# hitbc/deSAMBA

Measured on AMD Instinct MI355X. Metric: classified reads/s (50 kbp ONT reads, viral index), higher is better.
Workload: dtype u8/u64 integer

## Files before the change

__graft_entry__.py:

```python
import os
import subprocess
import sys

ROOT = os.path.dirname(os.path.abspath(__file__))
CSRC = os.path.join(ROOT, "desamba_amd", "csrc")
LIB = os.path.join(ROOT, "desamba_amd", "libdesamba_amd.so")
HIPCC = os.environ.get("HIPCC", "/opt/rocm/bin/hipcc")


def _run(cmd, cwd=None):
    print("+", " ".join(cmd), flush=True)
    subprocess.check_call(cmd, cwd=cwd)


def _newer(target, sources):
    if not os.path.exists(target):
        return False
    t = os.path.getmtime(target)
    return all(os.path.getmtime(s) <= t for s in sources)


def build():
    inc = os.path.join(ROOT, "include", "desamba_amd.h")
    H = lambda *names: [os.path.join(CSRC, f) for f in names] + [inc]
# ... 12 lines not shown
            o = os.path.join(objdir, src + (".o" if ku is None else ".k%d.o" % ku))
            if not _newer(o, [os.path.join(CSRC, src)] + hdrs) or os.environ.get("DSB_HIPCC_FLAGS"):
                jobs.append([HIPCC] + flags + ([] if ku is None else ["-DDSB_KUNIT=%d" % ku]) + ["-c", os.path.join(CSRC, src), "-o", o])
            objs.append(o)
    stage_dir = os.path.join(ROOT, "tests", "stage")
    stage_so = os.path.join(stage_dir, "libdsbstage.so")
    stage_src = os.path.join(stage_dir, "dsb_stage.hip")
    stage_forms = os.path.join(stage_dir, "dsb_stage_forms.h")
    if os.path.exists(stage_src) and os.path.exists(stage_forms) and (
            not _newer(stage_so, [stage_src, stage_forms] + H("dsb_classify_dev.h", "dsb_wave.h", "dsb_device.h")) or os.environ.get("DSB_HIPCC_FLAGS")):
        jobs.append([HIPCC] + flags + ["-I" + CSRC, "-I" + stage_dir, "-shared", "-o", stage_so, stage_src])
    if jobs:
        from concurrent.futures import ThreadPoolExecutor
        with ThreadPoolExecutor(max_workers=max(1, min(len(jobs), os.cpu_count() or 1))) as ex:
            list(ex.map(_run, jobs))
    stale = os.path.join(objdir, "dsb_gpu.hip.o")
    if os.path.exists(stale):
        os.remove(stale)
    deps = [os.path.join(CSRC, f) for f in ("dsb_classify_dev.h", "dsb_wave.h", "dsb_device.h", "dsb_host.h", "dsb_probe.h", "dsb_fastq_scan.h", "dsb_seed_scan.h", "dsb_build_impl.h", "dsb_build_host.h", "dsb_sam_fields.h")] + [inc]
    if not _newer(LIB, objs):
        _run([HIPCC, "--offload-arch=gfx950", "-shared", "-fPIC", "-o", LIB] + objs + ["-lz"])
    cli = os.path.join(ROOT, "desamba_amd", "bin", "deSAMBA")
    cli_src = os.path.join(CSRC, "desamba_main.c")
    ana_src = os.path.join(CSRC, "desamba_analysis.c")
    if os.path.exists(cli_src) and not _newer(cli, [cli_src, ana_src, LIB, os.path.join(CSRC, "dsb_fastq_scan.h")]):
        os.makedirs(os.path.dirname(cli), exist_ok=True)
        _run(["gcc", "-O2", "-std=gnu99", "-I" + os.path.join(ROOT, "include"), "-o", cli, cli_src, ana_src,
              "-L" + os.path.join(ROOT, "desamba_amd"), "-ldesamba_amd", "-Wl,-rpath,$ORIGIN/..", "-lpthread", "-lz", "-ldl"])
    sim = os.path.join(ROOT, "tools", "readsim")
    if not _newer(sim, [sim + ".c"]):
        _run(["gcc", "-O2", "-o", sim, sim + ".c", "-lm"])
    gen = os.path.join(ROOT, "tools", "libreadgen.so")
    if not _newer(gen, [os.path.join(ROOT, "tools", "readgen.c")]):
        _run(["gcc", "-O2", "-shared", "-fPIC", "-o", gen, os.path.join(ROOT, "tools", "readgen.c"), "-lpthread", "-lm"])
    gb = os.path.join(ROOT, "tools", "gather_bench")
    if not _newer(gb, [gb + ".hip"]):
        _run([HIPCC, "-O3", "--offload-arch=gfx950", gb + ".hip", "-o", gb])
    _run(["make", "-s", "-C", os.path.join(ROOT, "oracle"), "tools", "port", "ref", "ref_ubfree"])
    emu = os.path.join(ROOT, "tests", "emu", "libdsbemu.so")
    emu_src = os.path.join(ROOT, "tests", "emu", "emu_classify.cpp")
    emu_b = os.path.join(ROOT, "tests", "emu", "libdsbemu_build.so")
    emu_b_src = os.path.join(ROOT, "tests", "emu", "emu_build.cpp")
    if not _newer(emu_b, [emu_b_src] + H("dsb_build_impl.h", "dsb_build_parts.h", "dsb_build_host.h", "dsb_probe.h")):
        _run(["g++", "-std=c++17", "-O2", "-fno-strict-aliasing", "-fPIC", "-shared", "-I" + CSRC, "-I" + os.path.join(ROOT, "include"), "-o", emu_b, emu_b_src, "-lz"])
    emu_dir = os.path.join(ROOT, "tests", "emu")
    if os.path.exists(stage_forms):
        deps = deps + [stage_forms]
    if not _newer(emu, [emu_src, os.path.join(emu_dir, "dsb_emu_shim.h")] + deps):
        _run(["g++", "-std=c++17", "-O2", "-fno-strict-aliasing", "-fPIC", "-shared", "-DDSB_HOST_EMU", "-I" + CSRC, "-I" + os.path.join(ROOT, "include"), "-I" + emu_dir,
              "-o", emu, emu_src, os.path.join(CSRC, "dsb_index.cpp")])
    emu64 = os.path.join(emu_dir, "libdsbemu64.so")
    if not _newer(emu64, [emu_src, os.path.join(emu_dir, "dsb_emu_shim.h"), os.path.join(emu_dir, "emu_simt.cpp")] + deps):
        _run([os.path.join(emu_dir, "build_emu64.sh")])
    sys.path.insert(0, ROOT)
    import desamba_amd
    L = desamba_amd.lib()
    for name in desamba_amd.EXPORTS:
        getattr(L, name)
    print("build ok:", L.dsb_version().decode(), flush=True)


def demo_dir():
    d = os.path.join(ROOT, "data")
    if not os.access(d if os.path.isdir(d) else ROOT, os.W_OK):
        import tempfile
        d = os.path.join(tempfile.gettempdir(), "desamba_amd_data_%d" % os.getuid())
    d = os.path.join(d, "demo")
    subprocess.check_call([os.path.join(ROOT, "tools", "make_demo_index.sh"), d], stdout=sys.stderr)
    return d


def smoke():
    sys.path.insert(0, ROOT)
    sys.path.insert(0, os.path.join(ROOT, "tests"))
    import desamba_amd as D
    import oracle_lib as O
    d = demo_dir()
    idx = D.Index(os.path.join(d, "index"))
    ctx = D.Ctx(idx, 0)
    recs = D.read_fastq(os.path.join(d, "ERR1050068.fastq"), 32)
    reads = D.make_reads(recs)
    res = ctx.classify(reads)
    ora = O.Oracle(os.path.join(d, "index"))
    hist = 0
    for i, (name, seq, qual) in enumerate(recs):
        exp = ora.classify(seq, hist)
        hist = max(hist, len(seq))
        rr = res.reads[i]
        got = [res.hits[rr.first + k].key() for k in range(rr.n)]
        assert got == exp, "smoke: read %d differs from the oracle: %r vs %r" % (i, got, exp)
    t = ctx.timing()
    print("smoke ok: 32 reads bit-exact vs oracle; kernels ms: encode %.3f probe %.3f classify %.3f" % (t.encode_ms, t.seed_probe_ms, t.classify_ms), flush=True)
    ctx.close(); idx.close()


if __name__ == "__main__":
    build()
    if len(sys.argv) > 1 and sys.argv[1] == "smoke":
        smoke()
```

desamba_amd/__init__.py:

```python
import ctypes as C
import os

_HERE = os.path.dirname(os.path.abspath(__file__))
LIB_PATH = os.environ.get("DSB_LIB_PATH", os.path.join(_HERE, "libdesamba_amd.so"))

DSB_OK, DSB_EIO, DSB_ENODEV, DSB_ENOMEM, DSB_EINVAL, DSB_ECAP = 0, -1, -2, -3, -4, -5


class DsbOpts(C.Structure):
    _fields_ = [("L_min_matching", C.c_int), ("min_score", C.c_int), ("max_sec_N", C.c_int), ("n_slots", C.c_int),
                ("max_read_len", C.c_uint32), ("max_batch_reads", C.c_uint32), ("input_slots", C.c_int), ("reserved", C.c_int), ("max_batch_bases", C.c_uint64)]


class DsbRead(C.Structure):
    _fields_ = [("name", C.c_char_p), ("seq", C.c_char_p), ("qual", C.c_char_p), ("len", C.c_uint32)]


class DsbHit(C.Structure):
    _fields_ = [("ref_ID", C.c_uint32), ("t_st", C.c_uint32), ("t_ed", C.c_uint32), ("q_st", C.c_uint32), ("q_ed", C.c_uint32),
                ("sum_score", C.c_uint32), ("indel", C.c_uint32), ("direction", C.c_uint8), ("primary", C.c_uint8),
                ("pri_index", C.c_uint8), ("pad", C.c_uint8)]

    def key(self):
        return (self.ref_ID, self.t_st, self.t_ed, self.q_st, self.q_ed, self.sum_score, self.direction, self.primary, self.pri_index)


class DsbReadResult(C.Structure):
    _fields_ = [("first", C.c_uint32), ("n", C.c_uint32), ("status", C.c_int32), ("fast", C.c_uint32), ("device_us", C.c_uint32), ("n_anc", C.c_uint32)]


class DsbResult(C.Structure):
    _fields_ = [("reads", C.POINTER(DsbReadResult)), ("hits", C.POINTER(DsbHit)), ("n_hits", C.c_size_t)]


class DsbSeed(C.Structure):
    _fields_ = [("offset", C.c_uint32), ("len", C.c_uint32), ("top", C.c_uint8), ("pad", C.c_uint8 * 3)]


class DsbTiming(C.Structure):
    _fields_ = [("encode_ms", C.c_float), ("seed_probe_ms", C.c_float), ("classify_ms", C.c_float), ("total_ms", C.c_float),
                ("windows", C.c_uint64), ("probes_t1", C.c_uint64), ("bases", C.c_uint64),
                ("order_ms", C.c_float), ("tail_ms", C.c_float), ("n_early", C.c_uint32), ("n_retry", C.c_uint32),
                ("n_regrow", C.c_uint32), ("seed_scan", C.c_uint32),
                ("n_occ", C.c_uint64), ("n_mem", C.c_uint64), ("n_sa", C.c_uint64), ("ref_bases", C.c_uint64),
                ("main_occ", C.c_uint64), ("main_mem", C.c_uint64), ("main_sa", C.c_uint64), ("main_ref_bases", C.c_uint64),
                ("n_heavy_mw", C.c_uint32), ("n_requeue", C.c_uint32), ("upload_bytes", C.c_uint64),
                ("anc_pool_asked", C.c_uint64), ("anc_pool_cap", C.c_uint64)]


class DsbBuildStats(C.Structure):
    _fields_ = [(n, C.c_uint64) for n in ("n_bases", "n_refs", "n_kmer", "n_unitig", "n_rows")] + \
               [(n, C.c_double) for n in ("parse_s", "sort_s", "graph_s", "walk_s", "rows_s", "tables_s", "write_s", "total_s")] + \
               [(n, C.c_uint64) for n in ("budget_bytes", "peak_device_bytes")] + \
               [(n, C.c_uint32) for n in ("ranges_kmers", "ranges_unitig_numbers", "ranges_rows", "ranges_exist")] + \
               [("spilled_bytes", C.c_uint64)]


class DsbReadTaxon(C.Structure):
    _fields_ = [("taxid", C.c_uint32), ("score", C.c_uint32), ("len", C.c_uint32), ("mapq", C.c_uint8), ("flags", C.c_uint8), ("pad", C.c_uint16)]


DSB_TAXON_CLASSIFIED, DSB_TAXON_HOST = 1, 2


class DsbRefCoverage(C.Structure):
    _fields_ = [("numreads", C.c_uint64), ("covbases", C.c_uint64), ("aligned_bases", C.c_uint64), ("mapq_sum", C.c_uint64)]


COVERAGE_FIELDS = ("numreads", "covbases", "aligned_bases", "mapq_sum")


class DsbEmOpts(C.Structure):
    _fields_ = [("max_iter", C.c_uint32), ("reserved", C.c_uint32), ("tol", C.c_double)]


class DsbAbundanceSummary(C.Structure):
    _fields_ = [("reads", C.c_uint64), ("classified", C.c_uint64), ("classes", C.c_uint64), ("iterations", C.c_uint32),
                ("converged", C.c_uint32), ("max_change", C.c_double), ("min_permille", C.c_uint32), ("reserved", C.c_uint32)]


ABUNDANCE_DTYPE = [("numreads", "<u8"), ("uniqreads", "<u8"), ("est_reads", "<f8"), ("read_share", "<f8"), ("copy_share", "<f8")]


class DsbReadLca(C.Structure):
    _fields_ = [("taxid", C.c_uint32), ("score", C.c_uint32), ("n_pass", C.c_uint32), ("depth", C.c_uint16), ("flags", C.c_uint8), ("pad", C.c_uint8)]


DSB_LCA_CLASSIFIED, DSB_LCA_NO_TAXON, DSB_LCA_AMBIGUOUS = 1, 2, 4
LCA_DTYPE = [("taxid", "<u4"), ("score", "<u4"), ("n_pass", "<u4"), ("depth", "<u2"), ("flags", "u1"), ("pad", "u1")]
TAXON_COUNT_DTYPE = [("taxid", "<u4"), ("pad", "<u4"), ("clade_reads", "<u8"), ("direct_reads", "<u8")]


class DsbLcaSummary(C.Structure):
    _fields_ = [("reads", C.c_uint64), ("classified", C.c_uint64), ("no_taxon", C.c_uint64), ("ambiguous", C.c_uint64),
                ("min_permille", C.c_uint32), ("reserved", C.c_uint32)]


LCA_SUMMARY_FIELDS = ("reads", "classified", "no_taxon", "ambiguous", "min_permille")


# ... 722 lines not shown
```

desamba_amd/csrc/dsb_classify_dev.h:

```cpp
#include "dsb_device.h"

#ifndef DSB_GROUP
#define DSB_GROUP 64
#endif
#ifndef DSB_NS
#define DSB_NS dsb_g64
#endif

#ifndef DSB_DEV_COMMON
#define DSB_DEV_COMMON
#define MAXV(a,b) (((a) > (b))?(a):(b))
#define MINV(a,b) (((a) < (b))?(a):(b))
#define ABSV(a) (((a) > 0)?(a): (- (a)))
#define ABS_U(a,b) (((a) > (b))?((a) - (b)): ((b) - (a)))
#define D_FORWARD 1u
#define D_REVERSE 0u
#define D_U64MAX 0xffffffffffffffffULL
#define SPENT(w) (++(w).steps > (w).step_limit)
#define LSPENT(l) (++(l).lsteps > (l).step_limit)
#define TICK(w, k) do { if ((w).dbg) { uint64_t _t = DSB_CLOCK(); (w).tacc[k] += _t - (w).tlast; (w).tlast = _t; } } while (0)
#ifdef DSB_TIMERS
#define SUB0(w) do { if ((w).dbg) (w).tsub = DSB_CLOCK(); } while (0)
#define SUB1(w, k) do { if ((w).dbg) (w).tacc[k] += DSB_CLOCK() - (w).tsub; } while (0)
#define TX0(w, v) uint64_t v = (w).dbg ? DSB_CLOCK() : 0
#define TX1(w, k, v) do { if ((w).dbg) (w).tx[k] += DSB_CLOCK() - (v); } while (0)
#define TXC(w, k) do { if ((w).dbg) (w).tx[k] += 1; } while (0)
#else
#define SUB0(w) do { } while (0)
#define SUB1(w, k) do { } while (0)
#define TX0(w, v) do { } while (0)
#define TX1(w, k, v) do { } while (0)
#define TXC(w, k) do { } while (0)
#endif
#define MARK(w, code) do { if ((w).dbg && DSB_LANE == 0) { (w).dbg[0] = (code); (w).dbg[1] = (w).steps; } } while (0)
#ifdef DSB_LDS_DIET
#define DSB_WTAB_SLOTS 2176u
#else
#define DSB_WTAB_SLOTS 3072u
#endif
#define DSB_WTAB_MAXQ 2048u
#define DSB_WTAB_EMPTY 0xffffffffu
#endif

#ifndef DSB_BOOST_IF_HEAVY
#define DSB_BOOST_PREDS 300000u
#define DSB_MIDDLE_HEAVY_MIN 16384u
#ifndef DSB_LANE_STEPS
#define DSB_LANE_STEPS 256u
#endif
#define DSB_BOOST_IF_HEAVY(w) do { if (!(w).boosted && (w).dp_preds > DSB_BOOST_PREDS) { dsb_setprio3(); (w).boosted = 1; } } while (0)
#endif
#define DSB_HEAVY_CHECK(w) do { if ((w).heavy_limit && (w).dp_preds > (w).heavy_limit) { (w).status |= DSB_ST_HEAVY; (w).steps = (w).step_limit; } } while (0)

namespace DSB_NS {

#ifdef DSB_HOST_EMU
#include "dsb_emu_shim.h"
#else
#include "dsb_wave.h"
#endif

struct Cnt { lds_u32 *c; uint32_t uni; };
DV void cnt_add(const Cnt &k, int which, uint32_t v)
{
	if (k.uni && DSB_LANE != 0) return;
	lds_add(k.c + which, v);
}

#define DSB_MW_MAXW 8
#ifndef DSB_MW_MIN_PREDS
#define DSB_MW_MIN_PREDS 2048
#endif
struct DsbMw {
	uint32_t cmd;
	uint32_t n0, K;
	const DsbSms *sms;
	uint32_t nd_t[8], nd_q[8], nd_l[8];
	uint32_t cut[2][DSB_MW_MAXW];
	int32_t best[DSB_MW_MAXW][8];
};

#define DSB_DPB 8
struct DpBatch { uint32_t n0, K; int old_best[DSB_DPB]; uint32_t nd_t[DSB_DPB], nd_q[DSB_DPB], nd_l[DSB_DPB]; };
typedef DSB_LDS_AS DpBatch DpBatchL;

struct SDir { DsbSeed *seed_v; uint32_t l_seed_v; uint8_t *bin_read; const uint64_t *bits; uint32_t direction, total_score; };
struct SDirV { DsbSeed *seed_v; uint8_t *bin_read; uint32_t direction; };

struct WCtx {
	DsbXP x;
	uint8_t *bin; uint32_t L;
	DsbSeed *seeds;
	DsbMw *mw; int n_waves;
	const uint64_t *pk[2];
	DsbSeed *pre_seeds; const DsbSeedInfo *pre_info;
	DsbAnchor *anc, *anc_tmp; uint32_t n_anc, anc_cap;
	uint32_t anc_cap_main, hit_cap, step_limit;
	DsbAnchor *lane_anc; uint64_t *lane_spset; uint32_t *top_idx;
	DsbChain *hit, *hit_tmp; uint32_t n_hit;
	DsbSms *sms; uint32_t n_sms;
	uint32_t *wtab;
	DsbScHash *sc;
	DsbMem *mem_slow;
	uint64_t *spset;
	int *score_v;
	uint64_t *sortkey; uint32_t *sortidx;
	uint8_t *win_mid, *win_right, *win_left;
	uint32_t *red;
	uint32_t *round_info;
	uint32_t dp_preds;
	uint32_t heavy_limit;
	DpBatchL *dpb;
	uint4 *ring;
	int status; int max_read_l;
	int stage; int boosted; uint32_t sp_gen;
	Cnt k;
	uint32_t steps, lsteps; volatile uint32_t *dbg; uint64_t tacc[14], tlast, tsub, tx[10];
	SDir sd[2];
};
typedef DSB_LDS_AS WCtx WCtxL;
typedef DSB_LDS_AS SDir SDirL;
DV void sdir_set(SDirL *d, DsbSeed *seed_v, uint32_t l_seed_v, uint8_t *bin_read, const uint64_t *bits, uint32_t direction, uint32_t total_score)
{
	d->seed_v = seed_v; d->l_seed_v = l_seed_v; d->bin_read = bin_read; d->bits = bits; d->direction = direction; d->total_score = total_score;
}
DV void sdir_swap(SDirL *a, SDirL *b)
{
	DsbSeed *sv = a->seed_v; const uint32_t n = a->l_seed_v; uint8_t *br = a->bin_read; const uint64_t *bi = a->bits; const uint32_t di = a->direction, ts = a->total_score;
	sdir_set(a, b->seed_v, b->l_seed_v, b->bin_read, b->bits, b->direction, b->total_score);
	sdir_set(b, sv, n, br, bi, di, ts);
}
#define WK(w) (Cnt{(w).k.c, (w).k.uni})
struct LCtx { DsbAnchor *anc; uint32_t n_anc, anc_cap; uint64_t *spset; int status; uint32_t lsteps, step_limit, sp_gen; Cnt k; };
DV LCtx lctx_main(WCtxL &w)
{
	LCtx l; l.anc = w.anc; l.n_anc = w.n_anc; l.anc_cap = w.anc_cap; l.spset = w.spset; l.status = w.status; l.lsteps = w.lsteps; l.step_limit = w.step_limit;
	l.sp_gen = w.sp_gen; l.k.c = w.k.c; l.k.uni = w.k.uni;
	return l;
}
DV void lctx_done(WCtxL &w, const LCtx &l) { w.n_anc = l.n_anc; w.status = l.status; w.lsteps = l.lsteps; w.sp_gen = l.sp_gen; }

DV bool dsb_serial_lane() { wave_sync(); return DSB_LANE == 0; }
#define DSB_SERIAL(w) if (dsb_serial_lane())
DV void serial_end(WCtxL &) { wave_sync(); }

DV uint64_t d_hash64_1(uint64_t key)
{
	key = (~key + (key << 21)); key = key ^ key >> 24; key = ((key + (key << 3)) + (key << 8));
	key = key ^ key >> 14; key = ((key + (key << 2)) + (key << 4)); key = key ^ key >> 28; key = (key + (key << 31));
	return key;
}
DV uint64_t d_hash64_2(uint64_t key)
{
// ... 1728 lines not shown
DV void sdp_limits(const DsbSms &cs, uint32_t &lim_q, uint32_t &lim_t)
{
	if (MODE == 2) { lim_q = cs.q_pos + cs.len - 6 + 9 - 1; lim_t = cs.t_pos + cs.len - 6 + 9 - 1; }
	else { lim_q = cs.q_pos + 6; lim_t = cs.t_pos + 6; }
}
template <int MODE>
DV void sdp_judge(const DsbSms &cs, const DsbSms &ps, uint32_t lim_q, uint32_t lim_t, bool &skip, bool &brk, int &ns)
{
	brk = false; ns = 0;
	if (MODE == 2) {
		skip = (ps.q_pos < lim_q) || (ps.t_pos < lim_t);
		if (!skip) brk = (lim_t + 600 < ps.t_pos);
		if (!skip && !brk) {
			int indel = ps.q_pos - ps.t_pos - (lim_q - lim_t); int ai = ABSV(indel);
			if (ai > 200) skip = true;
			else {
				ns = ps.score + cs.len - (ai >> 3);
				if (lim_q + 6 > ps.q_pos || lim_t + 6 > ps.t_pos) { int oq = lim_q + 6 - ps.q_pos, ot = lim_t + 6 - ps.t_pos; ns -= MAXV(oq, ot); }
			}
		}
	} else {
		int pre_q_ed = ps.q_pos + ps.len + 9 - 1, pre_t_ed = ps.t_pos + ps.len + 9 - 1;
		skip = ((uint32_t)pre_q_ed > lim_q) || ((uint32_t)pre_t_ed > lim_t);
		if (!skip) brk = (ps.t_pos + 600 < lim_t);
		if (!skip && !brk) {
			int indel = ps.q_pos - ps.t_pos - (lim_q - lim_t); int ai = ABSV(indel);
			if (ai > 200) skip = true;
			else {
				ns = ps.score + cs.len - (ai >> 3);
				if ((uint32_t)pre_q_ed > cs.q_pos || (uint32_t)pre_t_ed > cs.t_pos) { int oq = pre_q_ed - cs.q_pos, ot = pre_t_ed - cs.t_pos; ns -= MAXV(oq, ot); }
			}
		}
	}
}

template <int MODE, bool RING>
DN void sdp_batch_old(WCtxL &w, DpBatchL &b)
{
	uint32_t lq[DSB_DPB], lt[DSB_DPB], dl[DSB_DPB], nq[DSB_DPB], nt[DSB_DPB], nl[DSB_DPB]; int best[DSB_DPB];
	uint32_t stopm = 0, preds = 0, wnm = 0;
#pragma unroll
	for (int j = 0; j < DSB_DPB; j++) {
		DsbSms ndj; ndj.t_pos = b.nd_t[j]; ndj.q_pos = b.nd_q[j]; ndj.len = b.nd_l[j]; ndj.score = 0;
		uint32_t q_, t_; sdp_limits<MODE>(ndj, q_, t_);
		lq[j] = DSB_RFL(q_); lt[j] = DSB_RFL(t_);
		dl[j] = lq[j] - lt[j]; nl[j] = DSB_RFL(ndj.len);
		if (MODE == 2) { nq[j] = lq[j] + 6; nt[j] = lt[j] + 6; } else { nq[j] = DSB_RFL(ndj.q_pos); nt[j] = DSB_RFL(ndj.t_pos); }
		best[j] = -2147483647 - 1;
		if ((uint32_t)j >= b.K) stopm |= 1u << j;
		if ((int)(lq[j] | lt[j] | nq[j] | nt[j] | (lt[j] + 600)) < 0) wnm |= 1u << j;
	}
	stopm = DSB_RFL(stopm); wnm = DSB_RFL(wnm);
	const int32_t n0 = (int32_t)b.n0;
	DsbSms nx[DSB_DP_UNROLL];
#define DSB_FETCH_PREDS(dst, hi_, ng_)                                                                          \
	_Pragma("unroll") for (int u = 0; u < DSB_DP_UNROLL; u++) {                                                 \
		if (u >= (ng_)) break;                                                                                   \
		int32_t pi = (hi_) - u * DSB_WAVE - DSB_LANE;                                                              \
		if (pi < 0) { dst[u].t_pos = 0; dst[u].q_pos = (MODE == 2) ? 0u : 0xfffffff0u; dst[u].len = 0; dst[u].score = 0; } \
		else if (RING && pi > n0 - DSB_RING) { uint4 r = ring_ld(w.ring, pi & (DSB_RING - 1)); dst[u].t_pos = r.x; dst[u].q_pos = r.y; dst[u].len = r.z; dst[u].score = r.w; } \
		else dst[u] = w.sms[pi];                                                                                 \
	}
	int ng = 1;
	if (n0 > 0) { DSB_FETCH_PREDS(nx, n0 - 1, ng) }
	for (int32_t hi = n0 - 1; hi >= 0;) {
		uint32_t A[DSB_DP_UNROLL], B[DSB_DP_UNROLL], C[DSB_DP_UNROLL], D[DSB_DP_UNROLL], S[DSB_DP_UNROLL]; bool wrapped[DSB_DP_UNROLL];
#pragma unroll
		for (int u = 0; u < DSB_DP_UNROLL; u++) {
			wrapped[u] = false; A[u] = B[u] = C[u] = D[u] = S[u] = 0;
			if (u >= ng) continue;
			int32_t pi = hi - u * DSB_WAVE - DSB_LANE;
			DsbSms ps = nx[u];
			if (MODE == 2) { A[u] = ps.q_pos; B[u] = ps.t_pos; C[u] = ps.t_pos; }
			else { A[u] = ps.q_pos + ps.len + 8; B[u] = ps.t_pos + ps.len + 8; C[u] = ps.t_pos + 600; }
			D[u] = ps.q_pos - ps.t_pos; S[u] = ps.score;
			if (pi < 0 && MODE != 2) A[u] = 0x7fffffffu;
			wrapped[u] = dsb_ballot64((int)(A[u] | B[u] | C[u]) < 0) != 0;
		}
		const int32_t hi_next = hi - ng * DSB_WAVE;
		if (ng == DSB_DP_UNROLL && hi_next >= 0) { DSB_FETCH_PREDS(nx, hi_next, DSB_DP_UNROLL) }
		const bool plain = wnm == 0 && !(wrapped[0] | wrapped[1] | wrapped[2] | wrapped[3]) && ng == DSB_DP_UNROLL;
		uint32_t redo = ~stopm & ((1u << DSB_DPB) - 1u);
		if (plain) {
#pragma unroll
			for (int j = 0; j < DSB_DPB; j++) {
				if ((stopm >> j) & 1u) continue;
				int tb = -2147483647 - 1; bool anyb = false;
#pragma unroll
				for (int u = 0; u < DSB_DP_UNROLL; u++) {
					const int oq = (MODE == 2) ? (int)(nq[j] - A[u]) : (int)(A[u] - nq[j]);
					const int ot = (MODE == 2) ? (int)(nt[j] - B[u]) : (int)(B[u] - nt[j]);
					const int indel = (int)(D[u] - dl[j]); const int ai = ABSV(indel);
					int ovl = MAXV(oq, ot); ovl = MAXV(ovl, 0);
					const bool skip = ovl > 6;
					const bool brk = !skip & ((MODE == 2) ? (lt[j] + 600 < C[u]) : (C[u] < lt[j]));
					const int ns = (int)(S[u] + nl[j] - (uint32_t)(ai >> 3) - (uint32_t)ovl);
					anyb |= brk;
					if (!skip & !brk & (ai <= 200) & (ns > tb)) tb = ns;
				}
				if (dsb_ballot64(anyb) == 0) { if (tb > best[j]) best[j] = tb; redo &= ~(1u << j); }
			}
		}
		preds += (uint32_t)ng * DSB_WAVE * (uint32_t)__builtin_popcount(~stopm & ((1u << DSB_DPB) - 1u));
		if (redo)
#pragma unroll
		for (int j = 0; j < DSB_DPB; j++) {
			if (!((redo >> j) & 1u)) continue;
#pragma unroll
			for (int u = 0; u < DSB_DP_UNROLL; u++) {
				if (u >= ng) break;
				if ((stopm >> j) & 1u) break;
				const int oq = (MODE == 2) ? (int)(nq[j] - A[u]) : (int)(A[u] - nq[j]);
				const int ot = (MODE == 2) ? (int)(nt[j] - B[u]) : (int)(B[u] - nt[j]);
				const int indel = (int)(D[u] - dl[j]); const int ai = ABSV(indel);
				bool skip, brk; int ns;
				if (wrapped[u] || ((wnm >> j) & 1u)) {
					bool ov;
					if (MODE == 2) { skip = (A[u] < lq[j]) | (B[u] < lt[j]); brk = !skip & (lt[j] + 600 < C[u]); ov = (nq[j] > A[u]) | (nt[j] > B[u]); }
					else { skip = (A[u] > lq[j]) | (B[u] > lt[j]); brk = !skip & (C[u] < lt[j]); ov = (A[u] > nq[j]) | (B[u] > nt[j]); }
					ns = (int)(S[u] + nl[j] - (uint32_t)(ai >> 3));
					if (ov) ns -= MAXV(oq, ot);
				} else {
					int ovl = MAXV(oq, ot); ovl = MAXV(ovl, 0);
					skip = ovl > 6;
					brk = !skip & ((MODE == 2) ? (lt[j] + 600 < C[u]) : (C[u] < lt[j]));
					ns = (int)(S[u] + nl[j] - (uint32_t)(ai >> 3) - (uint32_t)ovl);
				}
				bool ok = !skip & !brk & (ai <= 200);
				uint64_t bm = dsb_ballot64(brk);
				if (bm) {
					int first_brk = grp_first(brk);
					ok = ok & (DSB_LANE < first_brk);
					stopm |= 1u << j;
				}
				if (ok && ns > best[j]) best[j] = ns;
			}
		}
		if (stopm == (1u << DSB_DPB) - 1u) break;
		if (ng != DSB_DP_UNROLL && hi_next >= 0) { DSB_FETCH_PREDS(nx, hi_next, DSB_DP_UNROLL) }
		hi = hi_next; ng = DSB_DP_UNROLL;
	}
	w.dp_preds += preds;
	DSB_HEAVY_CHECK(w);
#pragma unroll
	for (int j = 0; j < DSB_DPB; j++) b.old_best[j] = ((uint32_t)j < b.K) ? grp_max_i(best[j]) : 0;
}

template <int MODE>
DN void sdp_batch_old_mw(DsbMw *mw, uint4 *ring, uint32_t *red, const int lane, const int wv, const int W, uint32_t *preds_out)
{
	uint32_t lq[DSB_DPB], lt[DSB_DPB], dl[DSB_DPB], nq[DSB_DPB], nt[DSB_DPB], nl[DSB_DPB]; int best[DSB_DPB];
	uint32_t stopm = 0, wnm = 0, preds = 0;
	const uint32_t K = mw->K; const DsbSms *const sms = mw->sms;
#pragma unroll
	for (int j = 0; j < DSB_DPB; j++) {
		DsbSms nd; nd.t_pos = mw->nd_t[j]; nd.q_pos = mw->nd_q[j]; nd.len = mw->nd_l[j]; nd.score = 0;
		uint32_t q_, t_; sdp_limits<MODE>(nd, q_, t_);
		lq[j] = DSB_RFL(q_); lt[j] = DSB_RFL(t_);
		dl[j] = lq[j] - lt[j]; nl[j] = DSB_RFL(nd.len);
		if (MODE == 2) { nq[j] = lq[j] + 6; nt[j] = lt[j] + 6; } else { nq[j] = DSB_RFL(nd.q_pos); nt[j] = DSB_RFL(nd.t_pos); }
		best[j] = -2147483647 - 1;
		if ((uint32_t)j >= K) stopm |= 1u << j;
		if ((int)(lq[j] | lt[j] | nq[j] | nt[j] | (lt[j] + 600)) < 0) wnm |= 1u << j;
	}
	stopm = DSB_RFL(stopm); wnm = DSB_RFL(wnm);
	const int32_t n0 = (int32_t)mw->n0;
	const int32_t step = DSB_DP_UNROLL * DSB_WAVE;
	DsbSms nx[DSB_DP_UNROLL];
#define DSB_FETCH_PREDS_MW(dst, hi_)                                                                            \
	_Pragma("unroll") for (int u = 0; u < DSB_DP_UNROLL; u++) {                                                 \
		int32_t pi = (hi_) - u * DSB_WAVE - lane;                                                                \
		if (pi < 0) { dst[u].t_pos = 0; dst[u].q_pos = (MODE == 2) ? 0u : 0xfffffff0u; dst[u].len = 0; dst[u].score = 0; } \
		else if (pi > n0 - DSB_RING) { uint4 r = ring_ld(ring, pi & (DSB_RING - 1)); dst[u].t_pos = r.x; dst[u].q_pos = r.y; dst[u].len = r.z; dst[u].score = r.w; } \
		else dst[u] = sms[pi];                                                                                   \
	}
	int32_t hi = n0 - 1 - wv * step;
	if (hi >= 0) { DSB_FETCH_PREDS_MW(nx, hi) }
	for (uint32_t round = 0;; round++, hi -= W * step) {
		int v[DSB_DPB]; uint32_t cutm = 0;
#pragma unroll
		for (int j = 0; j < DSB_DPB; j++) v[j] = -2147483647 - 1;
		if (hi >= 0) {
			uint32_t A[DSB_DP_UNROLL], B[DSB_DP_UNROLL], C[DSB_DP_UNROLL], D[DSB_DP_UNROLL], S[DSB_DP_UNROLL]; bool wrapped[DSB_DP_UNROLL];
#pragma unroll
			for (int u = 0; u < DSB_DP_UNROLL; u++) {
				int32_t pi = hi - u * DSB_WAVE - lane;
				DsbSms ps = nx[u];
				if (MODE == 2) { A[u] = ps.q_pos; B[u] = ps.t_pos; C[u] = ps.t_pos; }
				else { A[u] = ps.q_pos + ps.len + 8; B[u] = ps.t_pos + ps.len + 8; C[u] = ps.t_pos + 600; }
				D[u] = ps.q_pos - ps.t_pos; S[u] = ps.score;
				if (pi < 0 && MODE != 2) A[u] = 0x7fffffffu;
				wrapped[u] = dsb_ballot64((int)(A[u] | B[u] | C[u]) < 0) != 0;
			}
			if (hi - W * step >= 0) { DSB_FETCH_PREDS_MW(nx, hi - W * step) }
			const bool plain = wnm == 0 && !(wrapped[0] | wrapped[1] | wrapped[2] | wrapped[3]);
			uint32_t redo = ~stopm & ((1u << DSB_DPB) - 1u);
			if (plain) {
#pragma unroll
				for (int j = 0; j < DSB_DPB; j++) {
					if ((stopm >> j) & 1u) continue;
					int tb = -2147483647 - 1; bool anyb = false;
#pragma unroll
					for (int u = 0; u < DSB_DP_UNROLL; u++) {
						const int oq = (MODE == 2) ? (int)(nq[j] - A[u]) : (int)(A[u] - nq[j]);
						const int ot = (MODE == 2) ? (int)(nt[j] - B[u]) : (int)(B[u] - nt[j]);
						const int indel = (int)(D[u] - dl[j]); const int ai = ABSV(indel);
						int ovl = MAXV(oq, ot); ovl = MAXV(ovl, 0);
						const bool skip = ovl > 6;
						const bool brk = !skip & ((MODE == 2) ? (lt[j] + 600 < C[u]) : (C[u] < lt[j]));
						const int ns = (int)(S[u] + nl[j] - (uint32_t)(ai >> 3) - (uint32_t)ovl);
						anyb |= brk;
						if (!skip & !brk & (ai <= 200) & (ns > tb)) tb = ns;
					}
					if (dsb_ballot64(anyb) == 0) { v[j] = tb; redo &= ~(1u << j); }
				}
			}
			preds += DSB_DP_UNROLL * DSB_WAVE * (uint32_t)__builtin_popcount(~stopm & ((1u << DSB_DPB) - 1u));
			if (redo)
#pragma unroll
			for (int j = 0; j < DSB_DPB; j++) {
				if (!((redo >> j) & 1u)) continue;
#pragma unroll
				for (int u = 0; u < DSB_DP_UNROLL; u++) {
					if ((cutm >> j) & 1u) break;
					const int oq = (MODE == 2) ? (int)(nq[j] - A[u]) : (int)(A[u] - nq[j]);
					const int ot = (MODE == 2) ? (int)(nt[j] - B[u]) : (int)(B[u] - nt[j]);
					const int indel = (int)(D[u] - dl[j]); const int ai = ABSV(indel);
					bool skip, brk; int ns;
					if (wrapped[u] || ((wnm >> j) & 1u)) {
						bool ov;
						if (MODE == 2) { skip = (A[u] < lq[j]) | (B[u] < lt[j]); brk = !skip & (lt[j] + 600 < C[u]); ov = (nq[j] > A[u]) | (nt[j] > B[u]); }
						else { skip = (A[u] > lq[j]) | (B[u] > lt[j]); brk = !skip & (C[u] < lt[j]); ov = (A[u] > nq[j]) | (B[u] > nt[j]); }
						ns = (int)(S[u] + nl[j] - (uint32_t)(ai >> 3));
						if (ov) ns -= MAXV(oq, ot);
					} else {
						int ovl = MAXV(oq, ot); ovl = MAXV(ovl, 0);
						skip = ovl > 6;
						brk = !skip & ((MODE == 2) ? (lt[j] + 600 < C[u]) : (C[u] < lt[j]));
						ns = (int)(S[u] + nl[j] - (uint32_t)(ai >> 3) - (uint32_t)ovl);
					}
					bool ok = !skip & !brk & (ai <= 200);
					if (dsb_ballot64(brk)) { const int first_brk = grp_first(brk); ok = ok & (lane < first_brk); cutm |= 1u << j; }
					if (ok && ns > v[j]) v[j] = ns;
				}
			}
		}
		const uint32_t par = round & 1u;
		if (lane == 0) mw->cut[par][wv] = cutm;
		block_sync();
		uint32_t newer = 0, all = 0;
		for (int u = 0; u < W; u++) { const uint32_t c = mw->cut[par][u]; if (u < wv) newer |= c; all |= c; }
#pragma unroll
		for (int j = 0; j < DSB_DPB; j++) if (!(((stopm | newer) >> j) & 1u) && v[j] > best[j]) best[j] = v[j];
		stopm |= all;
		if (stopm == (1u << DSB_DPB) - 1u) break;
		if (n0 - 1 - (int32_t)(round + 1) * W * step < 0) break;
	}
#undef DSB_FETCH_PREDS_MW
#pragma unroll
	for (int j = 0; j < DSB_DPB; j++) { const int m = grp_max_i(best[j]); if (lane == 0) mw->best[wv][j] = m; }
	block_sync();
	if (preds_out) *preds_out = preds;
}

template <int MODE>
DV int sdp_best_pred_b(WCtxL &w, DpBatchL &b, const DsbSms &cs, int32_t cur, const NodeBlock &nb, const uint32_t n_sms, uint4 *const ring, uint32_t &steps, uint32_t &bn0, uint32_t &bK)
{
	if ((uint32_t)cur < bn0 || (uint32_t)cur >= bn0 + bK) {
		bn0 = (uint32_t)cur; bK = MINV((uint32_t)DSB_DPB, n_sms - (uint32_t)cur);
		b.n0 = bn0; b.K = bK;
		for (uint32_t j = 0; j < bK; j++) {
			const uint32_t idx = (uint32_t)cur + j;
			if (DSB_WAVE == 64 && idx >= nb.base && idx < nb.base + nb.valid) {
				const int src = (int)(idx - nb.base);
				b.nd_t[j] = dsb_shfl(nb.mine.t_pos, src); b.nd_q[j] = dsb_shfl(nb.mine.q_pos, src); b.nd_l[j] = dsb_shfl(nb.mine.len, src);
				continue;
			}
			const DsbSms g_ = w.sms[cur + j];
			b.nd_t[j] = g_.t_pos; b.nd_q[j] = g_.q_pos; b.nd_l[j] = g_.len;
		}
		if (w.mw && bn0 >= DSB_MW_MIN_PREDS) {
			DsbMw *mw = w.mw;
			if (DSB_LANE < DSB_DPB) { const int sj = (uint32_t)DSB_LANE < b.K ? DSB_LANE : 0; mw->nd_t[DSB_LANE] = b.nd_t[sj]; mw->nd_q[DSB_LANE] = b.nd_q[sj]; mw->nd_l[DSB_LANE] = b.nd_l[sj]; }
			if (DSB_LANE == 0) { mw->cmd = (uint32_t)MODE; mw->n0 = b.n0; mw->K = b.K; mw->sms = w.sms; }
			block_sync();
			uint32_t preds = 0;
			sdp_batch_old_mw<MODE>(mw, w.ring, w.red, DSB_LANE, 0, w.n_waves, &preds);
			w.dp_preds += preds;
			for (uint32_t j = 0; j < DSB_DPB; j++) { int m = -2147483647 - 1; for (int u = 0; u < w.n_waves; u++) m = MAXV(m, mw->best[u][j]); b.old_best[j] = j < b.K ? m : 0; }
		} else
		{ TX0(w, t_o); sdp_batch_old<MODE, true>(w, b); TX1(w, 2, t_o); TXC(w, 6); }
		if (w.status & DSB_ST_HEAVY) steps = w.step_limit;
		DSB_BOOST_IF_HEAVY(w);
	}
	int best = (int)cs.len; bool cut = false;
	uint32_t lim_q, lim_t; sdp_limits<MODE>(cs, lim_q, lim_t);
	const int32_t m = cur - (int32_t)bn0;
	for (int32_t base = 0; base < m && !cut; base += DSB_WAVE) {
		const int32_t l = base + DSB_LANE; const bool valid = l < m;
		bool skip = true, brk = false; int ns = 0;
		if (valid) {
			uint4 r = ring_ld(ring, (uint32_t)(cur - 1 - l) & (DSB_RING - 1)); DsbSms ps; ps.t_pos = r.x; ps.q_pos = r.y; ps.len = r.z; ps.score = r.w;
			sdp_judge<MODE>(cs, ps, lim_q, lim_t, skip, brk, ns);
		}
		const int fb = grp_first(valid && !skip && brk);
		const int mine = (valid && !skip && !brk && DSB_LANE < fb) ? ns : (-2147483647 - 1);
		const int mx = grp_max_i(mine);
		if (mx > best) best = mx;
		if (fb < DSB_WAVE) cut = true;
	}
	int ob = b.old_best[cur - (int32_t)bn0];
	if (!cut && ob > best) best = ob;
	return best;
}

#ifndef DSB_BLK_CHUNKS
#define DSB_BLK_CHUNKS 1
#endif
template <int MODE>
DN int sdp_block_scores(WCtxL &w, const uint32_t n0_, const uint32_t m_, const DsbSms cs)
{
	const uint32_t n0 = DSB_RFL(n0_), m = DSB_RFL(m_);
	const int lane = DSB_LANE; const DsbSms *const sms = w.sms;
	const bool mine = (uint32_t)lane < m;
	uint32_t lim_q, lim_t; sdp_limits<MODE>(cs, lim_q, lim_t);
	const uint32_t lq = lim_q, lt = lim_t, dl = lq - lt, nl = cs.len;
	const uint32_t nq = MODE == 2 ? lq + 6 : cs.q_pos, nt = MODE == 2 ? lt + 6 : cs.t_pos;
	const bool node_wrapped = dsb_ballot64(mine && (int)(lq | lt | nq | nt | (lt + 600)) < 0) != 0;
	int best = (int)cs.len; bool done = !mine;
	uint32_t preds = 0;
#define DSB_BLK_PLAIN(pt, pq, pl, psc, BRK, OK, NS)                                                                          \
	const uint32_t A_ = MODE == 2 ? (pq) : (pq) + (pl) + 8, B_ = MODE == 2 ? (pt) : (pt) + (pl) + 8, C_ = MODE == 2 ? (pt) : (pt) + 600; \
	const int oq_ = MODE == 2 ? (int)(nq - A_) : (int)(A_ - nq), ot_ = MODE == 2 ? (int)(nt - B_) : (int)(B_ - nt);          \
	const int in_ = (int)((pq) - (pt) - dl); const int ai_ = ABSV(in_);                                                       \
	int ov_ = MAXV(oq_, ot_); ov_ = MAXV(ov_, 0);                                                                             \
	const bool sk_ = ov_ > 6;                                                                                                 \
	const bool BRK = !sk_ & ((MODE == 2) ? (lt + 600 < C_) : (C_ < lt));                                                      \
	const int NS = (int)((psc) + nl - (uint32_t)(ai_ >> 3) - (uint32_t)ov_);                                                  \
	const bool OK = !sk_ & !BRK & (ai_ <= 200);
	TX0(w, t_old);
	int32_t hi = (int32_t)n0 - 1;
	bool all_done = false;
	for (int ch = 0; ch < DSB_BLK_CHUNKS && hi >= 0 && !all_done; ch++) {
		const int32_t pi = hi - lane;
		DsbSms o; o.t_pos = o.q_pos = o.len = o.score = 0;
		if (pi >= 0) o = sms[pi];
		const int cnt = hi + 1 < DSB_WAVE ? hi + 1 : DSB_WAVE;
		const uint32_t oA = MODE == 2 ? o.q_pos : o.q_pos + o.len + 8, oB = MODE == 2 ? o.t_pos : o.t_pos + o.len + 8, oC = MODE == 2 ? o.t_pos : o.t_pos + 600;
		const bool plain = !node_wrapped && dsb_ballot64(pi >= 0 && (int)(oA | oB | oC) < 0) == 0;
		if (plain) {
			for (int k = 0; k < cnt; k++) {
				const uint32_t pt = dsb_shfl(o.t_pos, k), pq = dsb_shfl(o.q_pos, k), pl = dsb_shfl(o.len, k), psc = dsb_shfl(o.score, k);
				DSB_BLK_PLAIN(pt, pq, pl, psc, brk, ok, ns)
				best = (!done & ok & (ns > best)) ? ns : best;
				done |= brk;
				preds += DSB_WAVE;
				if (dsb_ballot64(!done) == 0) { all_done = true; break; }
			}
		} else {
			for (int k = 0; k < cnt; k++) {
				DsbSms ps; ps.t_pos = dsb_shfl(o.t_pos, k); ps.q_pos = dsb_shfl(o.q_pos, k); ps.len = dsb_shfl(o.len, k); ps.score = dsb_shfl(o.score, k);
				bool skip, brk; int ns; sdp_judge<MODE>(cs, ps, lim_q, lim_t, skip, brk, ns);
				if (!done) { if (brk) done = true; else if (!skip && ns > best) best = ns; }
				preds += DSB_WAVE;
				if (dsb_ballot64(!done) == 0) { all_done = true; break; }
			}
		}
		hi -= DSB_WAVE;
	}
	uint64_t left = dsb_ballot64(!done);
	TX0(w, t_deep);
	if (hi >= 0 && left) {
		TXC(w, 7);
		DpBatchL &b = *w.dpb;
		while (left) {
			int id[DSB_DPB]; uint32_t K = 0;
			for (int j = 0; j < DSB_DPB; j++) { id[j] = -1; if (left) { id[j] = (int)__builtin_ctzll(left); left &= left - 1; K++; } }
			for (int j = 0; j < DSB_DPB; j++) if (lane == id[j]) { b.nd_t[j] = cs.t_pos; b.nd_q[j] = cs.q_pos; b.nd_l[j] = cs.len; }
			if (lane == 0) { b.n0 = (uint32_t)hi + 1; b.K = K; for (uint32_t j = K; j < DSB_DPB; j++) { b.nd_t[j] = 0; b.nd_q[j] = 0; b.nd_l[j] = 0; } }
			wave_sync();
			sdp_batch_old<MODE, false>(w, b);
			wave_sync();
			for (int j = 0; j < DSB_DPB; j++) if (lane == id[j]) { const int ob = b.old_best[j]; if (ob > best) best = ob; }
			wave_sync();
		}
	}
	TX1(w, 9, t_deep);
	TX1(w, 2, t_old);
	TX0(w, t_in);
	if (m > 1) {
		const uint32_t cA = MODE == 2 ? cs.q_pos : cs.q_pos + cs.len + 8, cB = MODE == 2 ? cs.t_pos : cs.t_pos + cs.len + 8, cC = MODE == 2 ? cs.t_pos : cs.t_pos + 600;
		const bool plain = !node_wrapped && dsb_ballot64(mine && (int)(cA | cB | cC) < 0) == 0;
		if (plain) {
			for (uint32_t c = 0; c + 1 < m; c++) {
				const uint32_t pt = dsb_shfl(cs.t_pos, (int)c), pq = dsb_shfl(cs.q_pos, (int)c), pl = dsb_shfl(cs.len, (int)c), psc = (uint32_t)dsb_shfl(best, (int)c);
				DSB_BLK_PLAIN(pt, pq, pl, psc, brk, ok, ns)
				const bool later = mine & ((uint32_t)lane > c);
				best = (later & brk) ? (int)cs.len : ((later & ok & (ns > best)) ? ns : best);
			}
		} else {
			for (uint32_t c = 0; c + 1 < m; c++) {
				DsbSms ps; ps.t_pos = dsb_shfl(cs.t_pos, (int)c); ps.q_pos = dsb_shfl(cs.q_pos, (int)c); ps.len = dsb_shfl(cs.len, (int)c); ps.score = (uint32_t)dsb_shfl(best, (int)c);
				if (mine && (uint32_t)lane > c) {
					bool skip, brk; int ns; sdp_judge<MODE>(cs, ps, lim_q, lim_t, skip, brk, ns);
					if (brk) best = (int)cs.len; else if (!skip && ns > best) best = ns;
				}
			}
		}
	}
#undef DSB_BLK_PLAIN
	TX1(w, 6, t_in);
	if (w.dbg) w.tx[8] += preds / DSB_WAVE;
	w.dp_preds += preds + m * DSB_WAVE;
	DSB_HEAVY_CHECK(w);
	return best;
}

DV void fill_window(const WCtxL &w, uint8_t *win, int n)
{
	for (int i = DSB_LANE; i < n; i += DSB_WAVE) win[i] = DSB_TPAD_VAL;
}

#ifdef DSB_LDS_DIET
#define DSB_GL_QW 9
#define DSB_GL_NODES 8
#else
#ifndef DSB_GL_QW
#define DSB_GL_QW 12
#define DSB_GL_NODES 12
#endif
#endif
static_assert((DSB_GL_QW + DSB_GL_NODES) * 64u * 8u <= 4u * DSB_WTAB_SLOTS, "gap_lane: its per-lane words live in the window table's LDS");
// ... 233 lines not shown
				const uint32_t nn = n_sms;
				DsbSms me; me.t_pos = me.q_pos = me.len = 0;
				if (lane == 0) me = first; else if ((uint32_t)lane == nn - 1) me = last; else if ((uint32_t)lane < nn) { if (mirror) { uint4 r = lnodes[lane]; me.t_pos = r.x; me.q_pos = r.y; me.len = r.z; } else me = S[lane]; }
				int mine = (lane == 0) ? score : (int)me.len;
				const uint32_t lim_q = me.q_pos + 6, lim_t = me.t_pos + 6;
				for (uint32_t pj = 0; pj + 1 < nn; pj++) {
					const uint32_t p_t = dsb_shfl(me.t_pos, (int)pj), p_q = dsb_shfl(me.q_pos, (int)pj), p_l = dsb_shfl(me.len, (int)pj); const int p_s = (int)dsb_shfl((uint32_t)mine, (int)pj);
					if ((uint32_t)lane > pj && (uint32_t)lane < nn) {
						const int pre_q_ed = (int)(p_q + p_l + 9 - 1), pre_t_ed = (int)(p_t + p_l + 9 - 1);
						if (!((uint32_t)pre_q_ed > lim_q) && !((uint32_t)pre_t_ed > lim_t)) {
							const int indel = (int)(p_q - p_t - (lim_q - lim_t)); const int ai = ABSV(indel);
							if (ai <= 200) {
								int ns = p_s + (int)me.len - (ai >> 3);
								if ((uint32_t)pre_q_ed > me.q_pos || (uint32_t)pre_t_ed > me.t_pos) { const int oq = pre_q_ed - (int)me.q_pos, ot = pre_t_ed - (int)me.t_pos; ns -= MAXV(oq, ot); }
								mine = MAXV(mine, ns);
							}
						}
					}
				}
				const int all_max = grp_max_i(((uint32_t)lane >= 1 && (uint32_t)lane < nn) ? mine : (-2147483647 - 1));
				score = MAXV(all_max, score);
			} else
			{
				S[0] = first; S[n_sms - 1].q_pos = last.q_pos; S[n_sms - 1].t_pos = last.t_pos; S[n_sms - 1].len = last.len;
				wave_sync();
				w.n_sms = n_sms;
				if (w.heavy_limit && n_sms >= DSB_MIDDLE_HEAVY_MIN) { w.status |= DSB_ST_HEAVY; w.steps = w.step_limit; w.n_sms = 0; return 0; }
				for (uint32_t ci = 1; ci < n_sms; ci++) {
					DsbSms cs = S[ci];
					int max_score = sdp_best_pred<0>(w, cs, (int32_t)ci);
					score = MAXV(max_score, score);
					S[ci].score = max_score;
				}
			}
		}
		whole_gain += score - score_before;
	}
	score = 10000 + (int)lane_gain + whole_gain + tail_len;
	w.n_sms = 0;
	return score - 10000;
}

DN int sdp_right_M2_mw(WCtxL &w, const uint8_t *q_str, int tbl, int key_len, DsbChain *c_st, int chain_ID, uint32_t l_read, DsbScHash *sc_hash, int score_ori)
{
	DsbXP x = w.x;
	score_ori += 10000;
	int total_max_score = score_ori, max_sms_id = 0;
	DsbChain *c_h = c_st + chain_ID, *combined;
	w.n_sms = 0;
	uint8_t *ref = w.win_right;
	fill_window(w, ref, 1000 + 128);
	wave_sync();
	DsbSms *p = push_sms(w);
	p->score = score_ori; p->q_pos = c_h->q_ed; p->t_pos = c_h->t_ed; p->len = 1 - 9;
	ring_put(w, 0, p->t_pos, p->q_pos, p->len, p->score);
	uint32_t best_t = c_h->t_ed, best_q = c_h->q_ed, best_len = (uint32_t)(1 - 9);
	NodeBlock nb; nb.base = 0; nb.valid = 0;
	DpBatchL &db = *w.dpb; db.n0 = 0; db.K = 0;
	uint32_t bn0 = 0, bK = 0;
	uint32_t current_sms = 1;
	uint64_t t_offset_global = x->refinfo[c_h->ref_ID].seq_offset, t_length = x->refinfo[c_h->ref_ID].seq_l;
	uint32_t c_t_offset = c_h->t_ed - 3;
	int last_search = false;
	uint32_t ch_q_st = c_h->q_st, ch_q_ed = c_h->q_ed;
	uint32_t steps = w.steps, n_sms = 1; const uint32_t step_limit = w.step_limit; DsbSms *const sms = w.sms; uint4 *const ring = w.ring;
	while (1) {
		if (++steps > step_limit) { w.status |= DSB_ST_TIMEOUT; break; }
		if (n_sms == current_sms) {
			uint32_t next_step = t_length - c_t_offset;
			if (next_step < 12) break;
			uint32_t max_search_ref;
			if (l_read - ch_q_ed < 600) {
				if (last_search == true) break;
				last_search = true;
				max_search_ref = l_read - ch_q_ed + 60;
			} else max_search_ref = t_length - c_t_offset;
			max_search_ref = MINV(600u, max_search_ref);
			get_ref_wave(x->refbin, x->ref_bases, DSB_LANE, ref, c_t_offset + t_offset_global, max_search_ref + 50); cnt_add(Cnt{w.k.c, 1u}, 3, max_search_ref + 50);
			wave_sync();
			int search_q_ed = (int)best_q + 1000;
			search_q_ed = MINV((uint32_t)search_q_ed, l_read);
			int search_q_st = MAXV((uint32_t)(search_q_ed - 2000), ch_q_st - 8);
			SUB0(w);
			sdp_match(w, search_q_st, search_q_ed, q_str, ref, max_search_ref, key_len, tbl, c_t_offset, true);
			SUB1(w, 10);
			c_t_offset += max_search_ref - 9 - 3;
			n_sms = w.n_sms;
			if (n_sms == current_sms) break;
			nb.valid = 0;
			if (node_get(w, nb, current_sms).t_pos > best_t + 1000) break;
		}
		DsbSms *c_sms = sms + current_sms;
		DsbSms cs = node_get(w, nb, current_sms); current_sms++;
		SUB0(w);
		int max_score = sdp_best_pred_b<1>(w, db, cs, (int32_t)current_sms - 1, nb, n_sms, ring, steps, bn0, bK);
		SUB1(w, 11);
		TXC(w, 8);
		c_sms->score = max_score;
		{ uint4 r_; r_.x = cs.t_pos; r_.y = cs.q_pos; r_.z = cs.len; r_.w = (uint32_t)max_score; ring_st(ring, (current_sms - 1) & (DSB_RING - 1), r_); }
		SUB0(w);
		bool comb = (int)cs.len >= 8 && combine_chain(c_st, chain_ID, sc_hash, cs.t_pos - cs.q_pos, false, cs.q_pos, &combined) == true;
		SUB1(w, 12);
		if (comb) {
			int c_len = cs.len;
			w.steps = steps;
			total_max_score = MAXV(score_ori, max_score) - c_len + sdp_middle_M2(w, combined->cur, q_str, tbl, key_len);
			steps = w.steps;
			ch_q_st = c_h->q_st; ch_q_ed = c_h->q_ed;
			score_ori = total_max_score; max_sms_id = 0;
			w.n_sms = 0;
			p = push_sms(w); n_sms = 1;
			p->score = total_max_score; p->q_pos = c_h->q_ed; p->t_pos = c_h->t_ed; p->len = -9;
			ring_put(w, 0, p->t_pos, p->q_pos, p->len, p->score);
			best_t = c_h->t_ed; best_q = c_h->q_ed; best_len = (uint32_t)(-9); nb.valid = 0; db.K = 0; bK = 0;
			current_sms = 1;
			c_t_offset = c_h->t_ed;
			continue;
		}
		if (total_max_score < max_score) { total_max_score = max_score; max_sms_id = current_sms - 1; best_t = cs.t_pos; best_q = cs.q_pos; best_len = cs.len; }
		if (cs.t_pos > best_t + 1000) break;
	}
	w.steps = steps;
	c_h->q_ed = best_q + best_len + 9;
	c_h->t_ed = best_t + best_len + 9;
	return total_max_score - 10000;
}

DN int sdp_left_M2_mw(WCtxL &w, const uint8_t *q_str, int tbl, int key_len, DsbChain *c_st, int chain_ID, uint32_t l_read, DsbScHash *sc_hash, int score_ori)
{
	DsbXP x = w.x;
	score_ori += 10000;
	int total_max_score = score_ori, max_sms_id = 0;
	DsbChain *c_h = c_st + chain_ID, *combined;
	w.n_sms = 0;
	uint8_t *ref = w.win_left;
	fill_window(w, ref, 1000 + 128);
	wave_sync();
	DsbSms *p = push_sms(w);
	p->score = score_ori; p->q_pos = c_h->q_st; p->t_pos = c_h->t_st;
	ring_put(w, 0, p->t_pos, p->q_pos, 0, p->score);
	uint32_t best_t = c_h->t_st, best_q = c_h->q_st;
	NodeBlock nb; nb.base = 0; nb.valid = 0;
	DpBatchL &db = *w.dpb; db.n0 = 0; db.K = 0;
	uint32_t bn0 = 0, bK = 0;
	uint32_t current_sms = 1;
	uint64_t t_offset_global = x->refinfo[c_h->ref_ID].seq_offset;
	uint32_t c_t_offset = c_h->t_st + 3;
	int last_search = false;
	uint32_t ch_q_st = c_h->q_st;
	uint32_t steps = w.steps, n_sms = 1; const uint32_t step_limit = w.step_limit; DsbSms *const sms = w.sms; uint4 *const ring = w.ring;
	while (1) {
		if (++steps > step_limit) { w.status |= DSB_ST_TIMEOUT; break; }
		if (n_sms == current_sms) {
			uint32_t next_step = c_t_offset;
			if (next_step < 12) break;
			uint32_t max_search_ref;
			if (ch_q_st < 600) {
				if (last_search == true) break;
				last_search = true;
				max_search_ref = ch_q_st + 60;
			} else max_search_ref = c_t_offset;
			max_search_ref = MINV(600u, max_search_ref);
			if (t_offset_global == 0 && c_t_offset < 50 + max_search_ref)
				{ get_ref_wave(x->refbin, x->ref_bases, DSB_LANE, ref, (int64_t)(c_t_offset + t_offset_global - max_search_ref), max_search_ref); cnt_add(Cnt{w.k.c, 1u}, 3, max_search_ref); }
			else
				{ get_ref_wave(x->refbin, x->ref_bases, DSB_LANE, ref, (int64_t)(c_t_offset + t_offset_global - max_search_ref - 50), max_search_ref + 50); cnt_add(Cnt{w.k.c, 1u}, 3, max_search_ref + 50); }
			wave_sync();
			int search_q_st = (int)best_q - 1000;
			search_q_st = MAXV(search_q_st, 0);
			int search_q_ed = MINV((uint32_t)(search_q_st + 2000), ch_q_st - 1);
			TX0(w, t_lm);
			sdp_match(w, search_q_st, search_q_ed, q_str, ref + 50, max_search_ref, key_len, tbl, c_t_offset - max_search_ref, false);
			TX1(w, 3, t_lm);
			c_t_offset = c_t_offset - max_search_ref + 9 + 3;
			n_sms = w.n_sms;
			if (n_sms == current_sms) break;
			nb.valid = 0;
			if (node_get(w, nb, current_sms).t_pos + 1000 < best_t) break;
		}
		DsbSms *c_sms = sms + current_sms;
		DsbSms cs = node_get(w, nb, current_sms); current_sms++;
		TX0(w, t_ld);
		int max_score = sdp_best_pred_b<2>(w, db, cs, (int32_t)current_sms - 1, nb, n_sms, ring, steps, bn0, bK);
		TX1(w, 4, t_ld);
		c_sms->score = max_score;
		{ uint4 r_; r_.x = cs.t_pos; r_.y = cs.q_pos; r_.z = cs.len; r_.w = (uint32_t)max_score; ring_st(ring, (current_sms - 1) & (DSB_RING - 1), r_); }
		if ((int)cs.len >= 8 && combine_chain(c_st, chain_ID, sc_hash, cs.t_pos - cs.q_pos, true, cs.q_pos + cs.len, &combined) == true) {
			int c_len = cs.len;
			w.steps = steps;
			total_max_score = MAXV(score_ori, max_score) - c_len + sdp_middle_M2(w, combined->cur, q_str, tbl, key_len);
			steps = w.steps;
			ch_q_st = c_h->q_st;
			score_ori = total_max_score; max_sms_id = 0;
			w.n_sms = 0;
			p = push_sms(w); n_sms = 1;
			p->score = total_max_score; p->q_pos = c_h->q_st; p->t_pos = c_h->t_st;
			ring_put(w, 0, p->t_pos, p->q_pos, 0, p->score);
			best_t = c_h->t_st; best_q = c_h->q_st; nb.valid = 0; db.K = 0; bK = 0;
			current_sms = 1;
			c_t_offset = c_h->t_st;
			continue;
		}
		if (total_max_score < max_score) { total_max_score = max_score; max_sms_id = current_sms - 1; best_t = cs.t_pos; best_q = cs.q_pos; }
		if (cs.t_pos + 1000 < best_t) break;
	}
	w.steps = steps;
	c_h->q_st = best_q;
	c_h->t_st = best_t;
	return total_max_score - 10000;
}

#define DSB_EXT_NEXT 0
#define DSB_EXT_STOP 1
#define DSB_EXT_MERGED 2
struct ExtState { int total_max_score; uint32_t best_t, best_q, best_len; uint32_t steps; int merge_score; uint32_t merge_len; DsbChain *combined; };
template <int MODE>
DV int ext_block(WCtxL &w, ExtState &e, const uint32_t n0, const uint32_t m, DsbChain *c_st, int chain_ID, DsbScHash *sc_hash, const uint32_t step_limit)
{
	const int lane = DSB_LANE; DsbSms *const sms = w.sms;
	const bool mine = (uint32_t)lane < m;
	DsbSms cs; cs.t_pos = cs.q_pos = cs.len = cs.score = 0;
	if (mine) cs = sms[n0 + lane];
	const int sc = sdp_block_scores<MODE>(w, n0, m, cs);
	if (mine) sms[n0 + lane].score = (uint32_t)sc;
	const bool cand = mine && (int)cs.len >= 8 && combine_test(c_st, chain_ID, sc_hash, (int)(cs.t_pos - cs.q_pos), MODE == 2, (int)(MODE == 2 ? cs.q_pos + cs.len : cs.q_pos));
	const uint64_t cmask = dsb_ballot64(cand);
	wave_sync();
	if (w.status & DSB_ST_HEAVY) { e.steps = step_limit; }
	DSB_BOOST_IF_HEAVY(w);
	for (uint32_t j = 0; j < m; j++) {
		if (++e.steps > step_limit) { w.status |= DSB_ST_TIMEOUT; return DSB_EXT_STOP; }
		const int s_j = dsb_shfl(sc, (int)j); const uint32_t t_j = dsb_shfl(cs.t_pos, (int)j);
		if ((cmask >> j) & 1ULL) {
			const uint32_t q_j = dsb_shfl(cs.q_pos, (int)j), l_j = dsb_shfl(cs.len, (int)j);
			if (combine_chain(c_st, chain_ID, sc_hash, (int)(t_j - q_j), MODE == 2, (int)(MODE == 2 ? q_j + l_j : q_j), &e.combined)) { e.merge_score = s_j; e.merge_len = l_j; return DSB_EXT_MERGED; }
		}
		if (e.total_max_score < s_j) { e.total_max_score = s_j; e.best_t = t_j; e.best_q = dsb_shfl(cs.q_pos, (int)j); e.best_len = dsb_shfl(cs.len, (int)j); }
		if (MODE == 1 ? (t_j > e.best_t + 1000) : (t_j + 1000 < e.best_t)) return DSB_EXT_STOP;
	}
	return DSB_EXT_NEXT;
}

DN int sdp_right_M2(WCtxL &w, const uint8_t *q_str, int tbl, int key_len, DsbChain *c_st, int chain_ID, uint32_t l_read, DsbScHash *sc_hash, int score_ori)
{
	DsbXP x = w.x;
	score_ori += 10000;
	DsbChain *c_h = c_st + chain_ID;
	w.n_sms = 0;
	uint8_t *ref = w.win_right;
	fill_window(w, ref, 1000 + 128);
	wave_sync();
	DsbSms *p = push_sms(w);
	p->score = score_ori; p->q_pos = c_h->q_ed; p->t_pos = c_h->t_ed; p->len = 1 - 9;
	ExtState e; e.total_max_score = score_ori; e.best_t = c_h->t_ed; e.best_q = c_h->q_ed; e.best_len = (uint32_t)(1 - 9);
	e.steps = w.steps; e.combined = nullptr; e.merge_score = 0; e.merge_len = 0;
	uint32_t current_sms = 1, n_sms = 1;
	uint64_t t_offset_global = x->refinfo[c_h->ref_ID].seq_offset, t_length = x->refinfo[c_h->ref_ID].seq_l;
	uint32_t c_t_offset = c_h->t_ed - 3;
	int last_search = false;
	uint32_t ch_q_st = c_h->q_st, ch_q_ed = c_h->q_ed;
	const uint32_t step_limit = w.step_limit; DsbSms *const sms = w.sms;
	wave_sync();
	while (1) {
		if (++e.steps > step_limit) { w.status |= DSB_ST_TIMEOUT; break; }
		if (n_sms == current_sms) {
			uint32_t next_step = t_length - c_t_offset;
			if (next_step < 12) break;
			uint32_t max_search_ref;
			if (l_read - ch_q_ed < 600) {
				if (last_search == true) break;
				last_search = true;
				max_search_ref = l_read - ch_q_ed + 60;
			} else max_search_ref = t_length - c_t_offset;
			max_search_ref = MINV(600u, max_search_ref);
			get_ref_wave(x->refbin, x->ref_bases, DSB_LANE, ref, c_t_offset + t_offset_global, max_search_ref + 50); cnt_add(Cnt{w.k.c, 1u}, 3, max_search_ref + 50);
			wave_sync();
			int search_q_ed = (int)e.best_q + 1000;
			search_q_ed = MINV((uint32_t)search_q_ed, l_read);
			int search_q_st = MAXV((uint32_t)(search_q_ed - 2000), ch_q_st - 8);
			SUB0(w);
			sdp_match(w, search_q_st, search_q_ed, q_str, ref, max_search_ref, key_len, tbl, c_t_offset, true);
			SUB1(w, 10);
			c_t_offset += max_search_ref - 9 - 3;
			n_sms = w.n_sms;
			if (n_sms == current_sms) break;
			if (sms[current_sms].t_pos > e.best_t + 1000) break;
		}
		const uint32_t m = MINV((uint32_t)DSB_WAVE, n_sms - current_sms);
		SUB0(w);
		const int how = ext_block<1>(w, e, current_sms, m, c_st, chain_ID, sc_hash, step_limit);
		SUB1(w, 11);
		if (how == DSB_EXT_STOP) break;
		if (how == DSB_EXT_MERGED) {
			w.steps = e.steps;
			e.total_max_score = MAXV(score_ori, e.merge_score) - (int)e.merge_len + sdp_middle_M2(w, e.combined->cur, q_str, tbl, key_len);
			e.steps = w.steps;
			ch_q_st = c_h->q_st; ch_q_ed = c_h->q_ed;
			score_ori = e.total_max_score;
			w.n_sms = 0;
			p = push_sms(w); n_sms = 1;
			p->score = e.total_max_score; p->q_pos = c_h->q_ed; p->t_pos = c_h->t_ed; p->len = -9;
			e.best_t = c_h->t_ed; e.best_q = c_h->q_ed; e.best_len = (uint32_t)(-9);
			current_sms = 1;
			c_t_offset = c_h->t_ed;
			wave_sync();
			continue;
		}
		current_sms += m;
	}
	w.steps = e.steps;
	c_h->q_ed = e.best_q + e.best_len + 9;
	c_h->t_ed = e.best_t + e.best_len + 9;
	return e.total_max_score - 10000;
}

DN int sdp_left_M2(WCtxL &w, const uint8_t *q_str, int tbl, int key_len, DsbChain *c_st, int chain_ID, uint32_t l_read, DsbScHash *sc_hash, int score_ori)
{
	DsbXP x = w.x;
	score_ori += 10000;
	DsbChain *c_h = c_st + chain_ID;
	w.n_sms = 0;
	uint8_t *ref = w.win_left;
	fill_window(w, ref, 1000 + 128);
	wave_sync();
	DsbSms *p = push_sms(w);
	p->score = score_ori; p->q_pos = c_h->q_st; p->t_pos = c_h->t_st; p->len = 0;
	ExtState e; e.total_max_score = score_ori; e.best_t = c_h->t_st; e.best_q = c_h->q_st; e.best_len = 0;
	e.steps = w.steps; e.combined = nullptr; e.merge_score = 0; e.merge_len = 0;
	uint32_t current_sms = 1, n_sms = 1;
	uint64_t t_offset_global = x->refinfo[c_h->ref_ID].seq_offset;
	uint32_t c_t_offset = c_h->t_st + 3;
	int last_search = false;
	uint32_t ch_q_st = c_h->q_st;
	const uint32_t step_limit = w.step_limit; DsbSms *const sms = w.sms;
	wave_sync();
	while (1) {
		if (++e.steps > step_limit) { w.status |= DSB_ST_TIMEOUT; break; }
		if (n_sms == current_sms) {
			uint32_t next_step = c_t_offset;
			if (next_step < 12) break;
			uint32_t max_search_ref;
			if (ch_q_st < 600) {
				if (last_search == true) break;
				last_search = true;
				max_search_ref = ch_q_st + 60;
			} else max_search_ref = c_t_offset;
			max_search_ref = MINV(600u, max_search_ref);
			if (t_offset_global == 0 && c_t_offset < 50 + max_search_ref)
				{ get_ref_wave(x->refbin, x->ref_bases, DSB_LANE, ref, (int64_t)(c_t_offset + t_offset_global - max_search_ref), max_search_ref); cnt_add(Cnt{w.k.c, 1u}, 3, max_search_ref); }
			else
				{ get_ref_wave(x->refbin, x->ref_bases, DSB_LANE, ref, (int64_t)(c_t_offset + t_offset_global - max_search_ref - 50), max_search_ref + 50); cnt_add(Cnt{w.k.c, 1u}, 3, max_search_ref + 50); }
			wave_sync();
			int search_q_st = (int)e.best_q - 1000;
			search_q_st = MAXV(search_q_st, 0);
			int search_q_ed = MINV((uint32_t)(search_q_st + 2000), ch_q_st - 1);
			TX0(w, t_lm);
			sdp_match(w, search_q_st, search_q_ed, q_str, ref + 50, max_search_ref, key_len, tbl, c_t_offset - max_search_ref, false);
			TX1(w, 3, t_lm);
			c_t_offset = c_t_offset - max_search_ref + 9 + 3;
			n_sms = w.n_sms;
			if (n_sms == current_sms) break;
			if (sms[current_sms].t_pos + 1000 < e.best_t) break;
		}
		const uint32_t m = MINV((uint32_t)DSB_WAVE, n_sms - current_sms);
		TX0(w, t_ld);
		const int how = ext_block<2>(w, e, current_sms, m, c_st, chain_ID, sc_hash, step_limit);
		TX1(w, 4, t_ld);
		if (how == DSB_EXT_STOP) break;
		if (how == DSB_EXT_MERGED) {
			w.steps = e.steps;
			e.total_max_score = MAXV(score_ori, e.merge_score) - (int)e.merge_len + sdp_middle_M2(w, e.combined->cur, q_str, tbl, key_len);
			e.steps = w.steps;
			ch_q_st = c_h->q_st;
			score_ori = e.total_max_score;
			w.n_sms = 0;
			p = push_sms(w); n_sms = 1;
			p->score = e.total_max_score; p->q_pos = c_h->q_st; p->t_pos = c_h->t_st; p->len = 0;
			e.best_t = c_h->t_st; e.best_q = c_h->q_st;
			current_sms = 1;
			c_t_offset = c_h->t_st;
			wave_sync();
			continue;
		}
		current_sms += m;
	}
	w.steps = e.steps;
	c_h->q_st = e.best_q;
	c_h->t_st = e.best_t;
	return e.total_max_score - 10000;
}

#ifdef DSB_EXT_PERNODE
#define DSB_EXT_MW(MW) true
#else
#define DSB_EXT_MW(MW) (MW)
#endif
template <bool MW>
DN void get_score_M2(WCtxL &w, SDirL *sd, uint32_t l_read, DsbScHash *sc_hash)
{
	TICK(w, 8);
	MARK(w, 50);
	int key_len = 0;
	MARK(w, 51);
	TICK(w, 4);
	DsbChain *H = w.hit;
	for (uint32_t i = 0; i < w.n_hit; i++) {
		if (H[i].sum_score == 0) continue;
		SDirL *csd = ((sd->direction == H[i].direction) ? 0 : 1) + sd;
		int tbl = (H[i].direction == D_FORWARD) ? 0 : 1;
		MARK(w, 52);
		int score = sdp_middle_M2(w, H[i].cur, csd->bin_read, tbl, key_len);
		MARK(w, 53);
		TICK(w, 5);
		score = DSB_EXT_MW(MW) ? sdp_right_M2_mw(w, csd->bin_read, tbl, key_len, H, i, l_read, sc_hash, score) : sdp_right_M2(w, csd->bin_read, tbl, key_len, H, i, l_read, sc_hash, score);
		MARK(w, 54);
		TICK(w, 6);
		score = DSB_EXT_MW(MW) ? sdp_left_M2_mw(w, csd->bin_read, tbl, key_len, H, i, l_read, sc_hash, score) : sdp_left_M2(w, csd->bin_read, tbl, key_len, H, i, l_read, sc_hash, score);
		MARK(w, 55);
		TICK(w, 7);
		H[i].sum_score = score;
	}
}

DV void small_score_head_cut(WCtxL &w)
{
	if (w.n_hit > 200) {
		uint32_t r = 200;
		for (; r < w.n_hit && w.hit[r].sum_score > 50; r++);
		w.n_hit = r;
	}
// ... 186 lines not shown
```

desamba_amd/csrc/dsb_ctx.h:

```cpp
#pragma once
#include <stdio.h>
#include <string.h>
#include <time.h>
#include <string>
#include "dsb_seed_scan.h"
#include "dsb_reductions.h"

#define HIPCHK(e) do { hipError_t _e = (e); if (_e != hipSuccess) { fprintf(stderr, "[desamba_amd] HIP error %s at %s:%d\n", hipGetErrorString(_e), __FILE__, __LINE__); return DSB_ENODEV; } } while (0)

struct DsbStaged;

struct InSlot {
	DsbReadDesc *d_rd = nullptr; char *d_ascii = nullptr; size_t cap_rd = 0, cap_ascii = 0;
	std::vector<DsbReadDesc> h_rd;
	size_t n_reads = 0; uint64_t n_words_total = 0, total_bases = 0, total_windows = 0, seed_entries = 0; uint32_t max_len = 0, min_len = 0;
	uint32_t *d_scan_order = nullptr; size_t cap_scan_order = 0;
	bool ragged = false;
	uint64_t upload_bytes = 0;
	bool packed = false;
};

struct UpStage { char *buf[2] = {nullptr, nullptr}; hipEvent_t ev[2] = {nullptr, nullptr}; bool used[2] = {false, false}; hipStream_t st = nullptr; };

struct DsbKnobs {
	bool upload_text = false;
	bool debug = false, upload_trace = false, no_turn = false, turn_whole_run = false, no_group = false, heavy_first_set = false;
	long hout_cap = 0, sms_cap = 0, anc_cap_rt = 0, upload_chunk_kb = 0, step_limit_rt = 0, group_head = -1;
	int upload_threads = 0, seed_scan = -1, heavy_mw = -1, heavy_first = 0;
	bool heavy_preds_set = false; uint32_t heavy_preds = 0;
	uint64_t em_hash_mask = ~0ull;
	bool anchor_kernel = true; long anc_pool_rt = 0;
	bool scan_look_set = false; DsbScanLook scan_look;
	std::string order_file;
};
inline bool g_upload_trace = false;

struct dsb_ctx {
	bool ek_dense = false;
	DsbKnobs knobs;
	dsb_index *idx = nullptr; int device = 0; hipStream_t stream = nullptr;
	DsbStaged *staged = nullptr; DsbDevIndex dx;
	std::vector<InSlot> in; int cur = 0;
	DsbWordDesc *d_wd = nullptr; uint8_t *d_bin = nullptr; uint64_t *d_pk = nullptr; uint64_t *d_bits = nullptr;
	size_t cap_wd = 0, cap_bin = 0, cap_pk = 0, cap_bits = 0;
	DsbReadOut *d_rout = nullptr; DsbHitOut *d_hout = nullptr; size_t cap_rout = 0, cap_hout = 0;
	unsigned int *d_counters = nullptr;
	DsbSlotArena arena; int n_slots = 0, n_extra = 0;
	DsbSlotArena arena_big; int n_slots_big = 0;
	DsbSlotArena arena_anc; int n_slots_anc = 0;
	DsbAncRec *d_arec = nullptr; DsbAnchor *d_apool = nullptr; size_t cap_arec = 0, cap_apool = 0;
	uint32_t hint_len = 0;
	unsigned mw_reads = 16; bool mw_grown = false; int mw_calm = 0;
	uint32_t *d_score = nullptr, *d_order = nullptr, *d_heavy = nullptr; size_t cap_score = 0, cap_order = 0, cap_heavy = 0;
	DsbSeed *d_seeds = nullptr; DsbSeedInfo *d_sinfo = nullptr; size_t cap_seeds = 0, cap_sinfo = 0;
	uint8_t *d_summ = nullptr; int summ_shift = 0;
	uint8_t *syn0 = nullptr, *syn1 = nullptr; bool seed_only = false;
	bool bits_valid = false, seeds_valid = false;
	unsigned n_early = 0;
	std::vector<DsbReadOut> h_rout; std::vector<DsbHitOut> h_hout;
	std::vector<dsb_read_result> res_reads;
	int hist_max = 0;
	hipEvent_t ev[4] = {nullptr, nullptr, nullptr, nullptr}; dsb_timing timing; unsigned long long p1 = 0;
	hipStream_t stream3 = nullptr; hipEvent_t ev_heavy3 = nullptr;
	hipStream_t stream2 = nullptr; hipEvent_t ev_order = nullptr, ev_heavy = nullptr, ev_hprobe = nullptr, ev_cls = nullptr, ev_cls_wait = nullptr;
	uint32_t *dbg_host = nullptr, *dbg_dev = nullptr;
	std::vector<UpStage> up; size_t up_chunk = 0;
	dsb_opts opts;
	DsbTaxa taxa; DsbCover cover; DsbEmStore em; DsbLca lca;
	dsb_ctx() { memset(&dx, 0, sizeof dx); memset(&arena, 0, sizeof arena); memset(&arena_big, 0, sizeof arena_big); memset(&arena_anc, 0, sizeof arena_anc); memset(&timing, 0, sizeof timing); memset(&opts, 0, sizeof opts); }
};

struct dsb_multi {
	dsb_index *idx = nullptr; std::vector<dsb_ctx *> ctx; uint32_t hist = 0;
	uint32_t chunk_reads_env = 0;
	std::vector<uint32_t> last_calls;
	std::vector<dsb_read_result> reads; std::vector<dsb_hit> hits;
	const dsb_taxonomy *tx = nullptr; std::vector<dsb_read_taxon> taxa; bool taxa_ok = false;
	std::vector<dsb_read_lca> lca; bool lca_on = false, lca_ok = false;
};

template <class T> static int grow(T **p, size_t *cap, size_t need)
{
	if (need <= *cap) return 0;
// ... 10 lines not shown
```

desamba_amd/csrc/dsb_device.h:

```cpp
#pragma once
#include <stddef.h>
#include <stdint.h>
#ifdef DSB_HOST_EMU
struct uint2 { uint32_t x, y; };
struct uint4 { uint32_t x, y, z, w; };
#else
#include <hip/hip_runtime.h>
#endif

struct DsbFmBlock {
	uint32_t cnt[4];
	uint64_t p0[2], p1[2];
	uint64_t sp[2];
};

struct DsbRefInfo { uint64_t seq_l, seq_offset; };

struct DsbHiLine { uint32_t base; uint16_t off[30]; };
#define DSB_HI_PER_LINE 29u
#define DSB_HI_DIV29(p) ((uint32_t)(((uint64_t)(p) * 2369637129ULL) >> 36))

struct DsbDevIndex {
	const uint8_t *ek0, *ek1; uint64_t ek_mask; int ek_len, single_base_max;
	const DsbFmBlock *fm; uint64_t bwt_len; uint64_t rank[6]; uint64_t dollar_pos; uint64_t dollar_row;
	const uint64_t *fm_sb;
	const uint64_t *hash_index;
	const DsbHiLine *hash_c;
	const uint2 *sa; const uint2 *uni; const uint64_t *refpos; const uint8_t *refbin; const DsbRefInfo *refinfo;
	uint64_t ref_bases;
	const int *qmem;
	const int *qlv;
	int filter_min_length, filter_min_score, filter_min_score_LV3;
	uint32_t sms_cap;
	uint32_t step_limit;
	uint32_t heavy_limit;
};

struct DsbSeed { uint32_t offset; uint16_t len, top; };
struct DsbSeedInfo { uint32_t n_seed[2], total[2]; uint32_t flags, pad; };

struct DsbAnchor {
	uint16_t mtch_len; int16_t score; uint8_t left_len, left_ED, rigt_len, rigt_ED;
	uint8_t direction, useless, duplicate, pad0; uint16_t seed_ID, chain_id;
	uint32_t ref_ID, ref_offset, index_in_read; int32_t pre;
	uint64_t global_offset;
};
struct DsbChain {
	uint32_t ref_ID; int32_t q_t_dis; uint32_t sum_score, anchor_number;
	uint8_t direction, with_top_anchor, primary, pri_index;
	uint32_t t_st, t_ed, q_st, q_ed, indel, chain_id; int32_t cur;
};
struct DsbSms { uint32_t t_pos, q_pos, len, score; };
struct DsbMem { int match_len; int sa_sp_l; uint64_t sp, sa_sp; int read_offset; int pad; };
struct DsbScHash { uint16_t next; uint16_t seed_ID; };

struct DsbHitOut { uint32_t ref_ID, t_st, t_ed, q_st, q_ed, sum_score, indel; uint8_t direction, primary, pri_index, pad; };
struct DsbReadOut { uint32_t first, n; int32_t status; uint32_t fast; uint32_t n_anc, pad; };
struct DsbAncRec { uint32_t off, n, lsteps, use; };

struct DsbReadDesc {
	uint64_t seq_off;
	uint64_t bin_off;
	uint64_t pk_off;
	uint64_t bit_off;
	uint32_t len;
	uint32_t n_win;
	uint32_t n_words;
	int32_t  hist_max;
	uint64_t seed_off;
};
struct DsbWordDesc { uint32_t read; uint32_t word; };

struct DsbSlotArena {
	uint8_t *base; size_t stride;
	size_t off_seeds, off_anc, off_anc_tmp, off_hit, off_hit_tmp, off_sms, off_sc, off_mem, off_spset, off_scorev,
	       off_sortkey, off_sortidx, off_win, off_lane_anc, off_lane_sp, off_top, off_round;
	uint32_t max_len;
	uint32_t sms_cap;
	uint32_t anc_cap, hit_cap;
};

#define DSB_QPAD_L 64
#define DSB_QPAD_R 192
#define DSB_QPAD_R_VAL 5
#define DSB_TPAD_VAL 4
#define DSB_ANC_CAP 8192
#define DSB_STEP_LIMIT 20000000u
#define DSB_HEAVY_PREDS 100000000u
#define DSB_HIT_CAP 4096
#define DSB_SMS_CAP 16384
static inline uint32_t dsb_sms_cap_for(uint32_t max_len) { uint32_t c = 2 * max_len; return c < DSB_SMS_CAP ? DSB_SMS_CAP : c; }
#define DSB_MEMSLOW_CAP (8 * 800 + 1 + 16)
#define DSB_SPSET_CAP 500
#define DSB_REFWIN 2176
#define DSB_REFWIN_FRONT 64

#define DSB_ST_ANC_OVF 1
#define DSB_ST_HIT_OVF 2
#define DSB_ST_SMS_OVF 4
#define DSB_ST_OUT_OVF 8
#define DSB_ST_TIMEOUT 16
#define DSB_ST_HEAVY 32
```

desamba_amd/csrc/dsb_gpu.hip:

```cpp
#include <hip/hip_runtime.h>
#include <stdint.h>
#include <stdio.h>
#include <string.h>
#include <stdlib.h>
#include <vector>
#include <string>
#include <unistd.h>
#include <fcntl.h>
#include <sys/mman.h>
#include <sys/stat.h>
#include "dsb_device.h"
#include "dsb_probe.h"
#include "dsb_seed_scan.h"
#define DSB_GROUP 64
#define DSB_NS dsb_g64
#include "dsb_classify_dev.h"
#undef DSB_GROUP
#undef DSB_NS
#include "dsb_host.h"
#include "dsb_sam_fields.h"

#if !defined(DSB_KUNIT)
#define DSB_UNIT_HAS(n) 1
#define DSB_UNIT_HOST 1
// ... 315 lines not shown
}
__device__ __forceinline__ uint32_t order_bucket(uint32_t s)
{
	s |= 1u;
	const uint32_t lg = 31u - (uint32_t)__clz((int)s);
	const uint32_t mant = lg >= 6u ? (s >> (lg - 6u)) & 63u : (s << (6u - lg)) & 63u;
	return lg * 64u + mant;
}
__global__ void __launch_bounds__(1024) k_order(const uint32_t *score, uint32_t n, uint32_t *order)
{
	__shared__ uint32_t hist[2048], start[2048];
	hist[threadIdx.x] = 0; hist[threadIdx.x + 1024] = 0;
	__syncthreads();
	for (uint32_t i = threadIdx.x; i < n; i += 1024) atomicAdd(&hist[order_bucket(score[i])], 1u);
	__syncthreads();
	if (threadIdx.x == 0) { uint32_t acc = 0; for (int b = 2047; b >= 0; b--) { start[b] = acc; acc += hist[b]; } }
	__syncthreads();
	for (uint32_t i = threadIdx.x; i < n; i += 1024) order[atomicAdd(&start[order_bucket(score[i])], 1u)] = i;
}

#endif

#ifndef DSB_WAVES_PER_EU
#define DSB_WAVES_PER_EU 3
#endif
#if DSB_UNIT_HAS(1) || DSB_UNIT_HAS(2) || DSB_UNIT_HAS(3)
__device__ __forceinline__ void classify_kernel_body(const DsbDevIndex &x, const DsbReadDesc *rd, uint32_t n_fixed, const unsigned int *n_ptr,
        const uint32_t *list, uint8_t *bin, const uint64_t *bits, const DsbSlotArena &ar, unsigned int *work_counter, DsbReadOut *rout,
        DsbHitOut *hout, unsigned int *hout_counter, uint32_t hout_cap, uint32_t *dbg, uint32_t item_base, uint32_t slot_base, unsigned long long *work_cnt, DsbSeed *seed_blob, const DsbSeedInfo *sinfo, const uint64_t *pk, uint32_t group_mode,
        const DsbAncRec *arec, const DsbAnchor *apool)
{
	const int lane = threadIdx.x;
	const uint32_t slot_id = slot_base + blockIdx.x;
	uint8_t *slot = ar.base + (size_t)slot_id * ar.stride;
	__shared__ DsbDevIndex sx;
	__shared__ uint4 lds_ring[DSB_RING];
	__shared__ __attribute__((aligned(16))) uint32_t lds_wtab[DSB_WTAB_SLOTS];
	__shared__ uint32_t lds_red[2];
	__shared__ unsigned int s_word;
	__shared__ uint32_t lds_cnt[4];
	__shared__ dsb_g64::DpBatch lds_dpb;
	if (lane < 4) lds_cnt[lane] = 0;
	if (lane == 0) sx = x;
	__syncthreads();
	__shared__ dsb_g64::WCtx s_w;
	dsb_g64::WCtxL &w = *(dsb_g64::WCtxL *)&s_w;
	w.ring = lds_ring; w.dpb = (dsb_g64::DpBatchL *)&lds_dpb; w.red = lds_red; w.k.c = (dsb_g64::lds_u32 *)lds_cnt; w.k.uni = 1;
	w.x = (dsb_g64::DsbXP)&sx; w.dbg = dbg ? dbg + 4 * slot_id : nullptr;
	for (int i = 0; i < 14; i++) w.tacc[i] = 0;
	for (int i = 0; i < 10; i++) w.tx[i] = 0;
	w.seeds = (DsbSeed *)(slot + ar.off_seeds);
	w.anc = (DsbAnchor *)(slot + ar.off_anc); w.anc_tmp = (DsbAnchor *)(slot + ar.off_anc_tmp);
	w.hit = (DsbChain *)(slot + ar.off_hit); w.hit_tmp = (DsbChain *)(slot + ar.off_hit_tmp);
	w.sms = (DsbSms *)(slot + ar.off_sms);
	w.sc = (DsbScHash *)(slot + ar.off_sc); w.wtab = lds_wtab;
	w.mem_slow = (DsbMem *)(slot + ar.off_mem);
	w.spset = (uint64_t *)(slot + ar.off_spset);
	w.score_v = (int *)(slot + ar.off_scorev);
	w.sortkey = (uint64_t *)(slot + ar.off_sortkey); w.sortidx = (uint32_t *)(slot + ar.off_sortidx);
	w.win_mid = slot + ar.off_win + DSB_REFWIN_FRONT; w.win_right = w.win_mid + DSB_REFWIN; w.win_left = w.win_right + DSB_REFWIN;
	w.lane_anc = (DsbAnchor *)(slot + ar.off_lane_anc); w.lane_spset = (uint64_t *)(slot + ar.off_lane_sp);
	w.top_idx = (uint32_t *)(slot + ar.off_top); w.round_info = (uint32_t *)(slot + ar.off_round);
	w.anc_cap = ar.anc_cap; w.anc_cap_main = ar.anc_cap; w.hit_cap = ar.hit_cap; w.step_limit = x.step_limit; w.heavy_limit = x.heavy_limit; w.sp_gen = 0; w.mw = nullptr; w.n_waves = 1;
	for (uint32_t i = lane; i < 64u * DSB_SPHASH; i += 64) w.lane_spset[i] = 0;
	for (uint32_t i = lane; i < DSB_SPHASH; i += 64) w.spset[i] = 0;
	__syncthreads();
	const unsigned int n_items = n_ptr ? *n_ptr : n_fixed;
	if (w.dbg && lane == 0) w.dbg[0] = 300;
	for (;;) {
		unsigned int n_grp = 1u;
		if (group_mode && seed_blob) n_grp = __hip_atomic_load(work_counter, __ATOMIC_RELAXED, __HIP_MEMORY_SCOPE_AGENT) >= group_mode ? 64u : 1u;
		n_grp = (unsigned int)__builtin_amdgcn_readfirstlane((int)n_grp);
		if (lane == 0) s_word = atomicAdd(work_counter, n_grp);
		__syncthreads();
		unsigned int k = s_word + item_base;
		__syncthreads();
		if (k >= n_items) {
			if (lane < 4 && lds_cnt[lane]) atomicAdd(work_cnt + lane, (unsigned long long)lds_cnt[lane]);
			if (w.dbg && lane == 0) { w.dbg[0] = 999; for (int i = 0; i < 14; i++) dbg[4 * 65536 + 14 * slot_id + i] += (uint32_t)(w.tacc[i] / 100); for (int i = 0; i < 10; i++) dbg[8 * 65536 + 10 * slot_id + i] += (uint32_t)(i < 6 ? w.tx[i] / 100 : w.tx[i]); }
			break;
		}
		uint32_t g_nanc = 0, g_ovf = 0;
		if (n_grp > 1) {
			const bool valid = k + lane < n_items;
			const unsigned int rl = valid ? (list ? list[k + lane] : k + lane) : 0u;
			const DsbReadDesc dl = rd[rl];
			uint64_t tg = w.dbg ? wall_clock64() : 0;
			dsb_g64::fast_classify_lane(w, valid, bin + dl.bin_off + DSB_QPAD_L, dl.len, seed_blob + dl.seed_off, sinfo + rl, &g_nanc, &g_ovf);
			if (w.dbg) w.tacc[1] += wall_clock64() - tg;
		}
		for (unsigned int pass = 0; pass < (n_grp > 1 ? 2u : 1u); pass++)
		for (unsigned int gl = 0; gl < n_grp; gl++) {
			const unsigned int pos = k + gl;
			if (pos >= n_items) break;
			bool have_anc = false;
			if (n_grp > 1) {
				const uint32_t ovf_l = dsb_g64::dsb_shfl(g_ovf, (int)gl);
				if ((ovf_l != 0) != (pass == 1)) continue;
				have_anc = !ovf_l;
			}
		unsigned int r = list ? list[pos] : pos;
		DsbReadDesc d = rd[r];
		uint64_t t_start = wall_clock64();
		uint64_t tacc0[14]; if (w.dbg) for (int i = 0; i < 14; i++) tacc0[i] = w.tacc[i];
		if (w.dbg && lane == 0) { w.dbg[2] = r; w.dbg[0] = 100; }
		w.bin = bin + d.bin_off + DSB_QPAD_L; w.L = d.len; w.status = 0; w.max_read_l = d.hist_max;
		w.pre_seeds = seed_blob ? seed_blob + d.seed_off : nullptr; w.pre_info = sinfo + r;
		w.pk[0] = pk + d.pk_off; w.pk[1] = w.pk[0] + ((d.len + 31) / 32 + 1);
		uint32_t anc_lsteps = 0;
		if (have_anc) {
			const uint32_t na = dsb_g64::dsb_shfl(g_nanc, (int)gl);
			const DsbAnchor *src = w.lane_anc + (size_t)gl * DSB_LANE_ANC_CAP;
			for (uint32_t i = lane; i < na; i += 64) w.anc[i] = src[i];
			w.n_anc = na;
			dsb_g64::wave_sync();
		} else if (arec) {
			const DsbAncRec ar_r = arec[r];
			if (ar_r.use) {
				const DsbAnchor *src = apool + ar_r.off;
				for (uint32_t i = lane; i < ar_r.n; i += 64) w.anc[i] = src[i];
				w.n_anc = ar_r.n; anc_lsteps = ar_r.lsteps; have_anc = true;
				dsb_g64::wave_sync();
			}
		}
		uint32_t fast = dsb_g64::classify_read<false>(w, bits + d.bit_off, bits + d.bit_off + d.n_words, have_anc, anc_lsteps);
		if (w.boosted) __builtin_amdgcn_s_setprio(0);
		if (w.status & DSB_ST_HEAVY) w.n_hit = 0;
		if (lane == 0) s_word = w.n_hit ? atomicAdd(hout_counter, w.n_hit) : 0u;
		__syncthreads();
		unsigned int first = s_word;
		__syncthreads();
		uint32_t n_out = w.n_hit;
		if (first + n_out > hout_cap) { w.status |= DSB_ST_OUT_OVF; n_out = 0; }
		for (uint32_t i = lane; i < n_out; i += 64) {
			DsbChain h = w.hit[i]; DsbHitOut o;
			o.ref_ID = h.ref_ID; o.t_st = h.t_st; o.t_ed = h.t_ed; o.q_st = h.q_st; o.q_ed = h.q_ed; o.sum_score = h.sum_score; o.indel = h.indel;
			o.direction = h.direction; o.primary = h.primary; o.pri_index = h.pri_index; o.pad = 0;
			hout[first + i] = o;
		}
		if (w.dbg && lane == 0) { w.dbg[0] = 200; if (r < 65536u) for (int i = 0; i < 14; i++) dbg[16 * 65536 + 14 * r + i] = (uint32_t)((w.tacc[i] - tacc0[i]) / 100); }
		if (lane == 0) { DsbReadOut ro; ro.first = first; ro.n = n_out; ro.status = w.status | (w.status ? (w.stage << 8) : 0);
			ro.fast = fast | ((uint32_t)((wall_clock64() - t_start) / 100) << 1); ro.n_anc = w.n_anc; ro.pad = 0; rout[r] = ro; }
		}
	}
}
#endif

#define DSB_CLASSIFY_ARGS DsbDevIndex x, const DsbReadDesc *rd, uint32_t n_fixed, const unsigned int *n_ptr, const uint32_t *list, uint8_t *bin, const uint64_t *bits, DsbSlotArena ar, \
        unsigned int *work_counter, DsbReadOut *rout, DsbHitOut *hout, unsigned int *hout_counter, uint32_t hout_cap, uint32_t *dbg, uint32_t item_base, uint32_t slot_base, unsigned long long *work_cnt, \
        DsbSeed *seed_blob, const DsbSeedInfo *sinfo, const uint64_t *pk, uint32_t group_mode, const DsbAncRec *arec, const DsbAnchor *apool
#define DSB_CLASSIFY_PASS x, rd, n_fixed, n_ptr, list, bin, bits, ar, work_counter, rout, hout, hout_counter, hout_cap, dbg, item_base, slot_base, work_cnt, seed_blob, sinfo, pk, group_mode, arec, apool
#if DSB_UNIT_HAS(1)
__global__ void __launch_bounds__(64, DSB_WAVES_PER_EU) k_classify(DSB_CLASSIFY_ARGS) { classify_kernel_body(DSB_CLASSIFY_PASS); }
#else
__global__ void k_classify(DSB_CLASSIFY_ARGS);
#endif
#if DSB_UNIT_HAS(2)
__global__ void __launch_bounds__(64, DSB_WAVES_PER_EU) k_classify_early(DSB_CLASSIFY_ARGS) { classify_kernel_body(DSB_CLASSIFY_PASS); }
#else
__global__ void k_classify_early(DSB_CLASSIFY_ARGS);
#endif
#if DSB_UNIT_HAS(3)
__global__ void __launch_bounds__(64, DSB_WAVES_PER_EU) k_classify_second(DSB_CLASSIFY_ARGS) { classify_kernel_body(DSB_CLASSIFY_PASS); }
#else
__global__ void k_classify_second(DSB_CLASSIFY_ARGS);
#endif

#ifndef DSB_ANCHOR_WPE
#define DSB_ANCHOR_WPE 5
#endif
#if DSB_UNIT_HAS(5)
__global__ void __launch_bounds__(64, DSB_ANCHOR_WPE) k_anchor(DsbDevIndex x, const DsbReadDesc *rd, uint32_t n_items, uint32_t item_base, const uint32_t *list,
        uint8_t *bin, DsbSlotArena ar, unsigned int *work_counter, DsbSeed *seed_blob, const DsbSeedInfo *sinfo, DsbAncRec *arec, DsbAnchor *apool,
        unsigned int *pool_counter, uint32_t pool_cap, unsigned long long *work_cnt)
{
	const int lane = threadIdx.x;
	uint8_t *slot = ar.base + (size_t)blockIdx.x * ar.stride;
	__shared__ DsbDevIndex sx;
	__shared__ __attribute__((aligned(16))) uint32_t lds_hist[128];
	__shared__ uint32_t lds_red[2];
	__shared__ unsigned int s_word;
	__shared__ uint32_t lds_cnt[4];
	if (lane < 4) lds_cnt[lane] = 0;
	if (lane == 0) sx = x;
	__syncthreads();
	__shared__ dsb_g64::WCtx s_w;
	dsb_g64::WCtxL &w = *(dsb_g64::WCtxL *)&s_w;
	w.red = lds_red; w.k.c = (dsb_g64::lds_u32 *)lds_cnt; w.k.uni = 1;
	w.x = (dsb_g64::DsbXP)&sx; w.dbg = nullptr; w.wtab = lds_hist; w.mw = nullptr; w.n_waves = 1;
	w.anc = (DsbAnchor *)(slot + ar.off_anc);
	w.spset = (uint64_t *)(slot + ar.off_spset);
	w.sortidx = (uint32_t *)(slot + ar.off_sortidx);
	w.lane_anc = (DsbAnchor *)(slot + ar.off_lane_anc); w.lane_spset = (uint64_t *)(slot + ar.off_lane_sp);
	w.top_idx = (uint32_t *)(slot + ar.off_top); w.round_info = (uint32_t *)(slot + ar.off_round);
	w.anc_cap = ar.anc_cap; w.anc_cap_main = ar.anc_cap; w.step_limit = x.step_limit; w.sp_gen = 0;
// ... 32 lines not shown
				const unsigned int off = s_word;
				__syncthreads();
				use = (uint64_t)off + na <= pool_cap;
				if (use) {
					for (uint32_t i = lane; i < na; i += 64) apool[off + i] = w.anc[i];
					rec.off = off; rec.n = na; rec.lsteps = w.lsteps; rec.use = 1u;
				}
			}
			if (!use && lane < 4) lds_cnt[lane] = cnt0;
			__syncthreads();
		}
		if (lane == 0) arec[r] = rec;
	}
}
#else
__global__ void k_anchor(DsbDevIndex x, const DsbReadDesc *rd, uint32_t n_items, uint32_t item_base, const uint32_t *list,
        uint8_t *bin, DsbSlotArena ar, unsigned int *work_counter, DsbSeed *seed_blob, const DsbSeedInfo *sinfo, DsbAncRec *arec, DsbAnchor *apool,
        unsigned int *pool_counter, uint32_t pool_cap, unsigned long long *work_cnt);
#endif



#if DSB_UNIT_HAS(4)
template <int MWW>
__global__ void __launch_bounds__(64 * MWW, DSB_WAVES_PER_EU) k_classify_heavy(DsbDevIndex x, const DsbReadDesc *rd, uint32_t n_fixed, const unsigned int *n_ptr,
        const uint32_t *list, uint8_t *bin, const uint64_t *bits, DsbSlotArena ar, unsigned int *work_counter, DsbReadOut *rout,
        DsbHitOut *hout, unsigned int *hout_counter, uint32_t hout_cap, uint32_t slot_base, unsigned long long *work_cnt, const uint64_t *pk,
        DsbSeed *seed_blob, const DsbSeedInfo *sinfo)
{
	const int lane = threadIdx.x & 63, wv = threadIdx.x >> 6;
	const uint32_t slot_id = slot_base + blockIdx.x;
	uint8_t *slot = ar.base + (size_t)slot_id * ar.stride;
	__shared__ DsbDevIndex sx;
	__shared__ uint4 lds_ring[DSB_RING];
	__shared__ __attribute__((aligned(16))) uint32_t lds_wtab[DSB_WTAB_SLOTS];
	__shared__ uint32_t lds_red[MWW + 1];
	__shared__ unsigned int s_word;
	__shared__ uint32_t lds_cnt[4];
	__shared__ dsb_g64::DpBatch lds_dpb;
	__shared__ dsb_g64::DsbMw mw;
	if (threadIdx.x < 4) lds_cnt[threadIdx.x] = 0;
	if (threadIdx.x == 0) { sx = x; mw.cmd = 0; }
	__syncthreads();
	__shared__ dsb_g64::WCtx s_w;
	dsb_g64::WCtxL &w = *(dsb_g64::WCtxL *)&s_w;
	if (wv == 0) {
		w.ring = lds_ring; w.dpb = (dsb_g64::DpBatchL *)&lds_dpb; w.red = lds_red; w.k.c = (dsb_g64::lds_u32 *)lds_cnt; w.k.uni = 1;
		w.x = (dsb_g64::DsbXP)&sx; w.dbg = nullptr;
		for (int i = 0; i < 14; i++) w.tacc[i] = 0;
		for (int i = 0; i < 10; i++) w.tx[i] = 0;
		w.seeds = (DsbSeed *)(slot + ar.off_seeds);
		w.anc = (DsbAnchor *)(slot + ar.off_anc); w.anc_tmp = (DsbAnchor *)(slot + ar.off_anc_tmp);
		w.hit = (DsbChain *)(slot + ar.off_hit); w.hit_tmp = (DsbChain *)(slot + ar.off_hit_tmp);
		w.sms = (DsbSms *)(slot + ar.off_sms);
		w.sc = (DsbScHash *)(slot + ar.off_sc); w.wtab = lds_wtab;
		w.mem_slow = (DsbMem *)(slot + ar.off_mem);
		w.spset = (uint64_t *)(slot + ar.off_spset);
		w.score_v = (int *)(slot + ar.off_scorev);
		w.sortkey = (uint64_t *)(slot + ar.off_sortkey); w.sortidx = (uint32_t *)(slot + ar.off_sortidx);
		w.win_mid = slot + ar.off_win + DSB_REFWIN_FRONT; w.win_right = w.win_mid + DSB_REFWIN; w.win_left = w.win_right + DSB_REFWIN;
		w.lane_anc = (DsbAnchor *)(slot + ar.off_lane_anc); w.lane_spset = (uint64_t *)(slot + ar.off_lane_sp);
		w.top_idx = (uint32_t *)(slot + ar.off_top); w.round_info = (uint32_t *)(slot + ar.off_round);
		w.anc_cap = ar.anc_cap; w.anc_cap_main = ar.anc_cap; w.hit_cap = ar.hit_cap; w.step_limit = x.step_limit; w.heavy_limit = 0; w.sp_gen = 0;
		w.mw = &mw; w.n_waves = MWW;
		for (uint32_t i = lane; i < 64u * DSB_SPHASH; i += 64) w.lane_spset[i] = 0;
		for (uint32_t i = lane; i < DSB_SPHASH; i += 64) w.spset[i] = 0;
	}
	__syncthreads();
	const unsigned int n_items = n_ptr ? *n_ptr : n_fixed;
	for (;;) {
		if (threadIdx.x == 0) s_word = atomicAdd(work_counter, 1u);
		__syncthreads();
		const unsigned int k = s_word;
		__syncthreads();
		if (k >= n_items) {
			if (threadIdx.x < 4 && lds_cnt[threadIdx.x]) atomicAdd(work_cnt + threadIdx.x, (unsigned long long)lds_cnt[threadIdx.x]);
			break;
		}
		const unsigned int r = list ? list[k] : k;
		if (wv == 0) {
			DsbReadDesc d = rd[r];
			const uint64_t t_start = wall_clock64();
			w.bin = bin + d.bin_off + DSB_QPAD_L; w.L = d.len; w.status = 0; w.max_read_l = d.hist_max;
			w.pre_seeds = seed_blob ? seed_blob + d.seed_off : nullptr; w.pre_info = sinfo + r;
			w.pk[0] = pk + d.pk_off; w.pk[1] = w.pk[0] + ((d.len + 31) / 32 + 1);
			const uint32_t fast = dsb_g64::classify_read<true>(w, bits + d.bit_off, bits + d.bit_off + d.n_words);
			if (w.boosted) __builtin_amdgcn_s_setprio(0);
			if (lane == 0) { mw.cmd = 3; s_word = w.n_hit ? atomicAdd(hout_counter, w.n_hit) : 0u; }
			__syncthreads();
			const unsigned int first = s_word;
			uint32_t n_out = w.n_hit;
			if (first + n_out > hout_cap) { w.status |= DSB_ST_OUT_OVF; n_out = 0; }
			for (uint32_t i = lane; i < n_out; i += 64) {
				DsbChain h = w.hit[i]; DsbHitOut o;
				o.ref_ID = h.ref_ID; o.t_st = h.t_st; o.t_ed = h.t_ed; o.q_st = h.q_st; o.q_ed = h.q_ed; o.sum_score = h.sum_score; o.indel = h.indel;
				o.direction = h.direction; o.primary = h.primary; o.pri_index = h.pri_index; o.pad = 0;
				hout[first + i] = o;
			}
			if (lane == 0) { DsbReadOut ro; ro.first = first; ro.n = n_out; ro.status = w.status | (w.status ? (w.stage << 8) : 0);
				ro.fast = fast | ((uint32_t)((wall_clock64() - t_start) / 100) << 1); ro.n_anc = w.n_anc; ro.pad = 0; rout[r] = ro; }
		} else {
			__builtin_amdgcn_s_setprio(3);
			for (;;) {
				__syncthreads();
				const uint32_t cmd = mw.cmd;
				if (cmd == 3) break;
				if (cmd == 1) dsb_g64::sdp_batch_old_mw<1>(&mw, lds_ring, lds_red, lane, wv, MWW, nullptr);
				else dsb_g64::sdp_batch_old_mw<2>(&mw, lds_ring, lds_red, lane, wv, MWW, nullptr);
			}
		}
	}
}
#if defined(DSB_KUNIT)
template __global__ void k_classify_heavy<8>(DsbDevIndex, const DsbReadDesc *, uint32_t, const unsigned int *, const uint32_t *, uint8_t *, const uint64_t *, DsbSlotArena, unsigned int *, DsbReadOut *, DsbHitOut *, unsigned int *, uint32_t, uint32_t, unsigned long long *, const uint64_t *, DsbSeed *, const DsbSeedInfo *);
#endif
#else
template <int MWW>
__global__ void k_classify_heavy(DsbDevIndex x, const DsbReadDesc *rd, uint32_t n_fixed, const unsigned int *n_ptr,
        const uint32_t *list, uint8_t *bin, const uint64_t *bits, DsbSlotArena ar, unsigned int *work_counter, DsbReadOut *rout,
        DsbHitOut *hout, unsigned int *hout_counter, uint32_t hout_cap, uint32_t slot_base, unsigned long long *work_cnt, const uint64_t *pk,
        DsbSeed *seed_blob, const DsbSeedInfo *sinfo);
#endif

#if DSB_UNIT_HOST
__global__ void k_collect_retry(const DsbReadOut *rout, uint32_t n, uint32_t *list, unsigned int *count, int mask, int clear_n)
{
	uint32_t i = blockIdx.x * 256 + threadIdx.x;
	if (i >= n) return;
	int st = rout[i].status & 0xff;
	if (st & mask) list[atomicAdd(count, 1u)] = i;
	(void)clear_n;
}

#include "dsb_ctx.h"
#include <mutex>
#include <thread>
#include <algorithm>

struct DsbStaged {
	const dsb_index *idx; int device; int refs;
	DsbDevIndex dx;
	std::vector<void *> allocs;
	uint8_t *d_summ; int summ_shift;
	bool ek_dense = false;
	std::mutex run_mu;
};
static std::mutex g_stage_mu;
static std::vector<DsbStaged *> g_staged;

template <class T> static int stage_upload(DsbStaged *s, const T *src, size_t n, const T **dst)
{
	void *p = nullptr;
	if (hipMalloc(&p, n * sizeof(T) + 256) != hipSuccess) return DSB_ENOMEM;
// ... 38 lines not shown
			}
		}
	}
	ST(stage_upload(s, h->fm, h->n_fm, &dx.fm));
	if (h->fm_sb) ST(stage_upload(s, h->fm_sb, h->n_fm_sb * 5, &dx.fm_sb));
	dx.bwt_len = h->bwt_len; memcpy(dx.rank, h->rank, sizeof dx.rank); dx.dollar_pos = h->dollar_pos; dx.dollar_row = h->dollar_row;
	if (h->hash_c) { ST(stage_upload(s, h->hash_c, (size_t)h->n_hash_c, &dx.hash_c)); dx.hash_index = nullptr; }
	else { ST(stage_upload(s, h->hash_index, ((size_t)1 << 26) + 1, &dx.hash_index)); dx.hash_c = nullptr; }
	ST(stage_upload(s, (const uint2 *)h->sa, h->sa_size, &dx.sa));
	ST(stage_upload(s, (const uint2 *)h->uni, h->n_uni + 1, &dx.uni));
	ST(stage_upload(s, h->refpos, h->n_refpos + 1, &dx.refpos));
	ST(stage_upload(s, h->refbin, h->n_refbin + 4096, &dx.refbin)); dx.ref_bases = h->n_refbin * 4;
	ST(stage_upload(s, h->refinfo, h->n_ref, &dx.refinfo));
	ST(stage_upload(s, h->Q_MEM, (size_t)2000, &dx.qmem));
	ST(stage_upload(s, &h->Q_LV[0][0], (size_t)400, &dx.qlv));
#undef ST
	if (rc) { stage_free(s); return rc; }
	*out = s;
	return 0;
}
static int stage_acquire(dsb_index *idx, int device, DsbStaged **out)
{
	std::lock_guard<std::mutex> g(g_stage_mu);
	for (DsbStaged *s : g_staged) if (s->idx == idx && s->device == device) { s->refs++; *out = s; return 0; }
	DsbStaged *s = nullptr; int rc = stage_build(idx, device, &s);
	if (rc) return rc;
	s->refs = 1; g_staged.push_back(s); *out = s;
	return 0;
}
static void stage_release(DsbStaged *s)
{
	std::lock_guard<std::mutex> g(g_stage_mu);
	if (--s->refs > 0) return;
	for (size_t i = 0; i < g_staged.size(); i++) if (g_staged[i] == s) { g_staged.erase(g_staged.begin() + i); break; }
	stage_free(s);
}

static void knobs_read(DsbKnobs &k)
{
	auto num = [](const char *name, long dflt) { const char *e = getenv(name); return e ? atol(e) : dflt; };
	k = DsbKnobs();
	k.debug = getenv("DSB_DEBUG") != nullptr; k.upload_trace = getenv("DSB_UPLOAD_TRACE") != nullptr;
	k.upload_text = getenv("DSB_UPLOAD_TEXT") != nullptr;
	k.no_turn = getenv("DSB_NO_TURN") != nullptr; k.turn_whole_run = getenv("DSB_TURN_WHOLE_RUN") != nullptr; k.no_group = getenv("DSB_NO_GROUP") != nullptr;
	k.hout_cap = num("DSB_HOUT_CAP", 0); if (getenv("DSB_HOUT_CAP") && k.hout_cap <= 0) k.hout_cap = 1;
	k.sms_cap = num("DSB_SMS_CAP", 0); if (getenv("DSB_SMS_CAP") && k.sms_cap < 64) k.sms_cap = 64;
	k.anc_cap_rt = num("DSB_ANC_CAP_RT", 0); if (getenv("DSB_ANC_CAP_RT")) { if (k.anc_cap_rt < 64) k.anc_cap_rt = 64; if (k.anc_cap_rt > DSB_ANC_CAP) k.anc_cap_rt = DSB_ANC_CAP; }
	k.upload_chunk_kb = num("DSB_UPLOAD_CHUNK_KB", 0); k.upload_threads = (int)num("DSB_UPLOAD_THREADS", 0);
	k.step_limit_rt = num("DSB_STEP_LIMIT_RT", 0); k.group_head = num("DSB_GROUP_HEAD", -1);
	k.seed_scan = getenv("DSB_SEED_SCAN") ? (num("DSB_SEED_SCAN", 0) != 0 ? 1 : 0) : -1;
	k.heavy_mw = getenv("DSB_HEAVY_MW") ? (int)num("DSB_HEAVY_MW", 0) : -1;
	k.heavy_first_set = getenv("DSB_HEAVY_FIRST") != nullptr; k.heavy_first = (int)num("DSB_HEAVY_FIRST", 0);
	k.anchor_kernel = num("DSB_ANCHOR_KERNEL", 1) != 0;
	if (getenv("DSB_EM_HASH_BITS")) { const long b = num("DSB_EM_HASH_BITS", 64); k.em_hash_mask = b >= 64 ? ~0ull : b < 1 ? 1ull : (1ull << b) - 1; }
	k.anc_pool_rt = num("DSB_ANC_POOL_RT", 0); if (getenv("DSB_ANC_POOL_RT") && k.anc_pool_rt < 1) k.anc_pool_rt = 1;
	if (const char *e = getenv("DSB_HEAVY_PREDS")) { k.heavy_preds_set = true; k.heavy_preds = (uint32_t)strtoul(e, nullptr, 10); }
	if (const char *e = getenv("DSB_ORDER_FILE")) k.order_file = e;
	k.scan_look_set = false;
	if (const char *e = getenv("DSB_SCAN_LOOK")) {
		int a = 0, b = 0, f = 0, st = 0;
		if (sscanf(e, "%d,%d,%d,%d", &a, &b, &f, &st) == 4 && a >= 1 && a <= DSB_SCAN_W && b >= 1 && b <= DSB_SCAN_W - 2 && f >= 1 && f <= DSB_SCAN_W && st >= 1 && st <= DSB_SCAN_W) {
			k.scan_look.after_seed = (uint8_t)a; k.scan_look.back_fwd = (uint8_t)b; k.scan_look.fwd_n = (uint8_t)f; k.scan_look.stride_n = (uint8_t)st; k.scan_look_set = true;
		}
	}
	g_upload_trace = k.upload_trace;
}


extern "C" int dsb_device_count(void)
{
	int n = 0;
	return hipGetDeviceCount(&n) == hipSuccess ? n : 0;
}

static int ensure_buffers(dsb_ctx *c, size_t n, uint32_t max_len, uint64_t bin_bytes, uint64_t pk_words, uint64_t bit_words, uint64_t seed_entries);
struct SeqView { const char *p; uint32_t len; };
static int upload_views(dsb_ctx *c, const SeqView *reads, size_t n, const char *ext_text = nullptr, size_t ext_len = 0, const uint64_t *ext_off = nullptr);
static int upload_stages(dsb_ctx *c, int T);
static int upload_threads(const dsb_ctx *c);

extern "C" void dsb_ctx_reload_env(dsb_ctx *c)
{
	if (!c) return;
	knobs_read(c->knobs);
}

extern "C" void dsb_ctx_destroy(dsb_ctx *c)
{
	if (!c) return;
	hipSetDevice(c->device);
	if (c->stream) hipStreamSynchronize(c->stream);
	if (c->stream2) hipStreamSynchronize(c->stream2);
	for (InSlot &s : c->in) { hipFree(s.d_rd); hipFree(s.d_ascii); hipFree(s.d_scan_order); }
	hipFree(c->d_wd); hipFree(c->d_bin); hipFree(c->d_pk); hipFree(c->d_bits);
	reductions_release(c);
	hipFree(c->d_rout); hipFree(c->d_hout); hipFree(c->d_counters); hipFree(c->arena.base); hipFree(c->arena_big.base); hipFree(c->arena_anc.base); hipFree(c->d_arec); hipFree(c->d_apool); hipFree(c->d_score); hipFree(c->d_order); hipFree(c->d_heavy); hipFree(c->d_seeds); hipFree(c->d_sinfo); hipFree(c->syn0); hipFree(c->syn1);
	if (c->dbg_host) hipHostFree(c->dbg_host);
	for (UpStage &u : c->up) { if (u.st) { hipStreamSynchronize(u.st); hipStreamDestroy(u.st); } for (int k = 0; k < 2; k++) { if (u.ev[k]) hipEventDestroy(u.ev[k]); if (u.buf[k]) hipHostFree(u.buf[k]); } }
	for (int i = 0; i < 4; i++) if (c->ev[i]) hipEventDestroy(c->ev[i]);
	if (c->ev_order) hipEventDestroy(c->ev_order);
	if (c->ev_cls) hipEventDestroy(c->ev_cls);
	if (c->ev_cls_wait) hipEventDestroy(c->ev_cls_wait);
	if (c->ev_heavy) hipEventDestroy(c->ev_heavy);
	if (c->ev_hprobe) hipEventDestroy(c->ev_hprobe);
	if (c->stream2) hipStreamDestroy(c->stream2);
	if (c->stream3) { hipStreamSynchronize(c->stream3); hipStreamDestroy(c->stream3); }
// ... 108 lines not shown
	if (hipGetDevice(&dev) != hipSuccess || hipDeviceGetPCIBusId(bdf, sizeof bdf, dev) != hipSuccess) return false;
	for (char *q = bdf; *q; q++) *q = (char)tolower(*q);
	char path[192]; snprintf(path, sizeof path, "/sys/bus/pci/devices/%s/numa_node", bdf);
	FILE *f = fopen(path, "r"); if (!f) return false;
	int node = -1; if (fscanf(f, "%d", &node) != 1) node = -1;
	fclose(f);
	if (node < 0) return false;
	snprintf(path, sizeof path, "/sys/devices/system/node/node%d/cpulist", node);
	f = fopen(path, "r"); if (!f) return false;
	char list[4096] = {0}; const bool got = fgets(list, sizeof list, f) != nullptr; fclose(f);
	if (!got) return false;
	CPU_ZERO(set); int n = 0;
	for (char *q = list; *q && *q != '\n';) {
		char *e; long a = strtol(q, &e, 10), b = a;
		if (e == q) break;
		if (*e == '-') { q = e + 1; b = strtol(q, &e, 10); }
		for (long c = a; c <= b && c < CPU_SETSIZE; c++) { CPU_SET((int)c, set); n++; }
		q = (*e == ',') ? e + 1 : e;
	}
	return n > 0;
}
extern "C" void *dsb_host_alloc(size_t bytes)
{
	cpu_set_t old, want; bool moved = false;
	if (!getenv("DSB_NO_NUMA") && sched_getaffinity(0, sizeof old, &old) == 0 && gpu_node_cpus(&want)) {
		cpu_set_t both; CPU_AND(&both, &old, &want);
		if (CPU_COUNT(&both) > 0) moved = sched_setaffinity(0, sizeof both, &both) == 0;
	}
	void *p = nullptr;
	const bool ok = hipHostMalloc(&p, bytes, hipHostMallocDefault) == hipSuccess;
	if (moved) sched_setaffinity(0, sizeof old, &old);
	return ok ? p : nullptr;
}
extern "C" void dsb_host_free(void *p) { if (p) hipHostFree(p); }

static size_t al256(size_t v) { return (v + 255) & ~(size_t)255; }

#define DSB_HEAVY_SLOTS 512
#define DSB_RETRY_SLOTS 64
#define DSB_RETRY_GROW 32
#define DSB_RETRY_MAX_NODES (8u << 20)
#define DSB_RETRY_ANC (8u * DSB_ANC_CAP)
#define DSB_RETRY_HIT (4u * DSB_HIT_CAP)
static size_t arena_layout(DsbSlotArena &a, uint32_t max_len, int group, uint32_t sms_cap, uint32_t anc_cap, uint32_t hit_cap)
{
	size_t o = 0; const size_t f = hit_cap ? 1 : 0;
	a.max_len = max_len; a.sms_cap = sms_cap; a.anc_cap = anc_cap; a.hit_cap = hit_cap;
	a.off_seeds = o;   o += f * al256(((size_t)(max_len >> 1) + 64) * sizeof(DsbSeed));
	a.off_anc = o;     o += al256((size_t)anc_cap * sizeof(DsbAnchor));
	a.off_anc_tmp = o; o += f * al256((size_t)anc_cap * sizeof(DsbAnchor));
	a.off_hit = o;     o += al256((size_t)hit_cap * sizeof(DsbChain));
	a.off_hit_tmp = o; o += al256((size_t)hit_cap * sizeof(DsbChain));
	a.off_sms = o;     o += f * al256((size_t)sms_cap * sizeof(DsbSms));
	a.off_sc = o;      o += f * al256((size_t)(256 + 2 * 400 + 64) * sizeof(DsbScHash));
	a.off_mem = o;     o += f * al256((size_t)DSB_MEMSLOW_CAP * sizeof(DsbMem));
	a.off_spset = o;   o += al256((size_t)DSB_SPHASH * 8);
	a.off_scorev = o;  o += f * al256((size_t)1024 * sizeof(int));
	a.off_sortkey = o; o += f * al256((size_t)2 * anc_cap * sizeof(uint64_t));
	a.off_sortidx = o; o += al256((size_t)2 * anc_cap * sizeof(uint32_t));
	a.off_win = o;     o += f * al256((size_t)3 * DSB_REFWIN + DSB_REFWIN_FRONT);
	a.off_lane_anc = o; o += al256((size_t)group * DSB_LANE_ANC_CAP * sizeof(DsbAnchor));
	a.off_lane_sp = o;  o += al256((size_t)group * DSB_SPHASH * 8);
	a.off_top = o;      o += al256(((size_t)(max_len >> 1) + 64) * 4);
	a.off_round = o;    o += al256(((size_t)(max_len >> 1) + 64) * 4);
	a.stride = al256(o);
	return a.stride;
}
static int size_arena(DsbSlotArena &a, int *cur_slots, uint32_t max_len, int want_slots, int min_slots, uint32_t sms_cap, uint32_t anc_cap, uint32_t hit_cap,
                      int extra_slots, size_t budget, bool exact_cap = false, bool check_only = false, int *cur_extra = nullptr)
{
	const int have_extra = cur_extra ? *cur_extra : extra_slots;
	const bool fits = a.base && a.max_len >= max_len && (exact_cap ? a.sms_cap == sms_cap : a.sms_cap >= sms_cap) && have_extra >= extra_slots;
	const bool oversized = a.base && a.max_len > 4 * (uint64_t)max_len + 65536 && a.stride * ((size_t)*cur_slots + have_extra) > ((size_t)4 << 30);
	if (fits && !oversized && (*cur_slots >= want_slots || a.max_len > max_len)) return 0;
	if (check_only) return 1;
	if (g_upload_trace) fprintf(stderr, "[upload] an arena is (re)built: has max_len %u, %d + %d slots, sms_cap %u; wanted max_len %u, %d + %d slots, sms_cap %u%s\n", a.base ? a.max_len : 0u, *cur_slots, have_extra, a.base ? a.sms_cap : 0u, max_len, want_slots, extra_slots, sms_cap, oversized ? " (oversized)" : "");
	if (a.base && !oversized && a.max_len > max_len) max_len = a.max_len;
	if (a.base) { hipFree(a.base); a.base = nullptr; budget += a.stride * ((size_t)*cur_slots + have_extra); }
	DsbSlotArena n = a;
	const size_t stride = arena_layout(n, max_len, 64, sms_cap, anc_cap, hit_cap);
	int slots = want_slots;
	while (slots > min_slots && stride * ((size_t)slots + extra_slots) > budget) slots = slots * 3 / 4 > min_slots ? slots * 3 / 4 : min_slots;
	while (cur_extra && extra_slots > 0 && stride * ((size_t)slots + extra_slots) > budget) extra_slots /= 2;
	for (;;) {
		if (hipMalloc((void **)&n.base, stride * ((size_t)slots + extra_slots)) == hipSuccess) break;
		(void)hipGetLastError();
		n.base = nullptr;
		if (slots <= min_slots && !(cur_extra && extra_slots > 0)) { a.base = nullptr; *cur_slots = 0; if (cur_extra) *cur_extra = 0; return DSB_ENOMEM; }
		if (slots > min_slots) slots = slots / 2 > min_slots ? slots / 2 : min_slots; else extra_slots /= 2;
	}
	a = n; *cur_slots = slots; if (cur_extra) *cur_extra = extra_slots;
	return 0;
}

static int ensure_buffers(dsb_ctx *c, size_t n, uint32_t max_len, uint64_t bin_bytes, uint64_t pk_words, uint64_t bit_words, uint64_t seed_entries)
{
	int rc;
	if ((rc = grow(&c->d_seeds, &c->cap_seeds, (size_t)seed_entries + 64))) return rc;
	if ((rc = grow(&c->d_sinfo, &c->cap_sinfo, n + 1))) return rc;
	if ((rc = grow(&c->d_wd, &c->cap_wd, (size_t)bit_words + 1))) return rc;
	if ((rc = grow(&c->d_bin, &c->cap_bin, (size_t)bin_bytes + 256))) return rc;
	if ((rc = grow(&c->d_pk, &c->cap_pk, (size_t)pk_words + 8))) return rc;
	if ((rc = grow(&c->d_bits, &c->cap_bits, (size_t)bit_words + 8))) return rc;
	if ((rc = grow(&c->d_rout, &c->cap_rout, n + 1))) return rc;
	size_t want_hout = 16 * n + 4096;
	if (c->knobs.hout_cap) want_hout = (size_t)c->knobs.hout_cap;
// ... 259 lines not shown
                            bool pre_seeds, const DsbAncRec *arec = nullptr, const DsbAnchor *apool = nullptr)
{
	hipLaunchKernelGGL(kern, dim3(grid), dim3(64), 0, st, dx, (const DsbReadDesc *)s.d_rd, n_fixed, n_ptr, list, c->d_bin, (const uint64_t *)c->d_bits, ar, work_counter,
	                   c->d_rout, c->d_hout, c->d_counters + 1, (uint32_t)c->cap_hout, dbg, item_base, slot_base, (unsigned long long *)(c->d_counters + 16 + 8 * cnt_set),
	                   pre_seeds ? c->d_seeds : nullptr, (const DsbSeedInfo *)c->d_sinfo, (const uint64_t *)c->d_pk, (uint32_t)((pre_seeds && s.max_len <= DSB_GROUP_MAX_LEN && !c->knobs.no_group) ? (c->knobs.group_head >= 0 ? (unsigned)c->knobs.group_head : 8u * grid) : 0u), arec, apool);
}

static int batch_run_locked(dsb_ctx *c, std::unique_lock<std::mutex> *turn);
extern "C" int dsb_batch_run(dsb_ctx *c)
{
	if (!c) return DSB_EINVAL;
	if (c->staged && !c->knobs.no_turn) { std::unique_lock<std::mutex> g(c->staged->run_mu); return batch_run_locked(c, &g); }
	return batch_run_locked(c, nullptr);
}
static int batch_run_locked(dsb_ctx *c, std::unique_lock<std::mutex> *turn)
{
	HIPCHK(hipSetDevice(c->device));
	InSlot &s = c->in[c->cur];
	size_t n = s.n_reads;
	memset(&c->timing, 0, sizeof c->timing);
	c->timing.upload_bytes = s.upload_bytes;
	c->taxa.run = c->taxa.tx != nullptr && n == 0; c->taxa.done = false;
	c->lca.run = c->lca.d_direct != nullptr && n == 0; c->lca.done = false;
	if (n == 0) return DSB_OK;
	HIPCHK(hipMemsetAsync(c->d_counters, 0, 256, c->stream));
	HIPCHK(hipEventRecord(c->ev[0], c->stream));
	if (s.packed) hipLaunchKernelGGL(k_encode_bytes_pk, dim3((unsigned)n), dim3(256), 0, c->stream, s.d_rd, (const uint8_t *)s.d_ascii, c->d_bin);
	else hipLaunchKernelGGL(k_encode_bytes, dim3((unsigned)n), dim3(256), 0, c->stream, s.d_rd, s.d_ascii, c->d_bin);
	hipLaunchKernelGGL(k_encode_pack, dim3((unsigned)n), dim3(256), 0, c->stream, s.d_rd, c->d_bin, c->d_pk);
	HIPCHK(hipEventRecord(c->ev[1], c->stream));
	const bool dbg = c->knobs.debug && c->dbg_dev;
	if (dbg) { HIPCHK(hipStreamSynchronize(c->stream)); fprintf(stderr, "[dsb] encode done\n"); }
	hipLaunchKernelGGL(k_repeat_score, dim3((unsigned)n), dim3(256), 0, c->stream, s.d_rd, c->d_pk, c->d_score);
	hipLaunchKernelGGL(k_order, dim3(1), dim3(1024), 0, c->stream, c->d_score, (uint32_t)n, c->d_order);
	if (const char *of = c->knobs.order_file.empty() ? nullptr : c->knobs.order_file.c_str()) {
		std::vector<uint32_t> ord(n); FILE *f = fopen(of, "rb");
		if (f && fread(ord.data(), 4, n, f) == n) HIPCHK(hipMemcpyAsync(c->d_order, ord.data(), n * 4, hipMemcpyHostToDevice, c->stream));
		if (f) fclose(f);
		HIPCHK(hipStreamSynchronize(c->stream));
	}
	HIPCHK(hipEventRecord(c->ev_order, c->stream));
	unsigned n_heavy = 0;
	if (!dbg && s.n_words_total && !c->seed_only) {
		n_heavy = c->knobs.heavy_first_set ? (unsigned)c->knobs.heavy_first : (n >= 4096 ? (unsigned)(n / 64) : 0u);
		if (n_heavy > (unsigned)c->n_extra) n_heavy = (unsigned)c->n_extra;
		if (n_heavy > n / 2) n_heavy = (unsigned)(n / 2);
	}
	c->n_early = n_heavy;
	bool use_scan = n >= 2048;
	if (c->knobs.seed_scan >= 0) use_scan = c->knobs.seed_scan != 0;
	c->bits_valid = !use_scan; c->seeds_valid = use_scan;
	uint32_t step_limit = DSB_STEP_LIMIT;
	if (c->knobs.step_limit_rt > 0) step_limit = (uint32_t)c->knobs.step_limit_rt;
	DsbDevIndex dx1 = c->dx; dx1.sms_cap = c->arena.sms_cap; dx1.step_limit = step_limit;
	dx1.heavy_limit = DSB_HEAVY_PREDS;
	if (dbg) dx1.heavy_limit = 0;
	if (c->knobs.heavy_preds_set) dx1.heavy_limit = c->knobs.heavy_preds;
	if (n_heavy) {
		hipLaunchKernelGGL(k_seed_probe_reads, dim3(n_heavy * DSB_HPROBE_SPLIT), dim3(256), 0, c->stream, c->dx, (const DsbReadDesc *)s.d_rd, (const uint32_t *)c->d_order, c->d_pk, c->d_bits, c->d_summ, c->summ_shift);
		HIPCHK(hipEventRecord(c->ev_hprobe, c->stream));
		HIPCHK(hipEventRecord(c->ev_order, c->stream));
		unsigned n_mw = c->mw_reads;
		if (c->knobs.heavy_mw >= 0) n_mw = (unsigned)c->knobs.heavy_mw;
		if (n_mw > n_heavy) n_mw = n_heavy;
		c->timing.n_heavy_mw = n_mw;
		if (n_mw) {
			HIPCHK(hipStreamWaitEvent(c->stream3, c->ev_hprobe, 0));
			hipLaunchKernelGGL(k_classify_heavy<8>, dim3(n_mw), dim3(64 * 8), 0, c->stream3, dx1, (const DsbReadDesc *)s.d_rd, (uint32_t)n_mw, (const unsigned int *)nullptr, (const uint32_t *)c->d_order, c->d_bin,
			                   (const uint64_t *)c->d_bits, c->arena, c->d_counters + 10, c->d_rout, c->d_hout, c->d_counters + 1, (uint32_t)c->cap_hout, (uint32_t)c->n_slots,
			                   (unsigned long long *)(c->d_counters + 16 + 8), (const uint64_t *)c->d_pk, (DsbSeed *)nullptr, (const DsbSeedInfo *)c->d_sinfo);
			HIPCHK(hipEventRecord(c->ev_heavy3, c->stream3));
		}
		HIPCHK(hipStreamWaitEvent(c->stream2, c->ev_hprobe, 0));
		if (n_heavy > n_mw)
			launch_classify(k_classify_early, c, c->stream2, n_heavy - n_mw, dx1, s, (uint32_t)n_heavy, nullptr, (const uint32_t *)c->d_order, c->arena, c->d_counters + 4, nullptr, n_mw, (uint32_t)c->n_slots + n_mw, 1, false);
		HIPCHK(hipEventRecord(c->ev_heavy, c->stream2));
	}
	if (use_scan) {
		hipLaunchKernelGGL(k_seed_scan, dim3((unsigned)((2 * n + 255) / 256)), dim3(256), 0, c->stream, c->dx, (const DsbReadDesc *)s.d_rd, (const uint32_t *)(s.ragged ? s.d_scan_order : nullptr),
		                   (uint32_t)n, (const uint64_t *)c->d_pk, c->d_seeds, c->d_sinfo, (const uint8_t *)c->d_summ, c->summ_shift, (unsigned long long *)(c->d_counters + 40),
		                   c->knobs.scan_look_set ? c->knobs.scan_look : dsb_scan_look_for((c->dx.ek_mask + 1) / 8, c->ek_dense));
	} else if (s.n_words_total) {
		uint64_t waves = (s.n_words_total + DSB_PROBE_UN - 1) / DSB_PROBE_UN; unsigned blocks = (unsigned)((waves + 3) / 4);
		if (blocks > 256u * 32u) blocks = 256u * 32u;
		hipLaunchKernelGGL(k_build_wd, dim3((unsigned)n), dim3(256), 0, c->stream, s.d_rd, c->d_wd);
		hipLaunchKernelGGL(k_seed_probe, dim3(blocks), dim3(256), 0, c->stream, c->dx, (const DsbReadDesc *)s.d_rd, (const DsbWordDesc *)c->d_wd, s.n_words_total, c->d_pk, c->d_bits,
		                   (unsigned long long *)(c->d_counters + 2), c->d_summ, c->summ_shift);
	}
	HIPCHK(hipEventRecord(c->ev[2], c->stream));
	if (c->seed_only) {
		HIPCHK(hipStreamSynchronize(c->stream));
		hipEventElapsedTime(&c->timing.encode_ms, c->ev[0], c->ev[1]);
		hipEventElapsedTime(&c->timing.order_ms, c->ev[1], c->ev_order);
		hipEventElapsedTime(&c->timing.seed_probe_ms, c->ev_order, c->ev[2]);
		unsigned long long pc[2] = {0, 0};
		HIPCHK(hipMemcpy(pc, use_scan ? c->d_counters + 40 : c->d_counters + 2, use_scan ? 16 : 8, hipMemcpyDeviceToHost));
		c->timing.windows = use_scan ? pc[0] : s.total_windows; c->timing.probes_t1 = use_scan ? pc[1] : pc[0]; c->timing.bases = s.total_bases;
		c->timing.seed_scan = use_scan ? 1 : 0; c->timing.total_ms = c->timing.encode_ms + c->timing.order_ms + c->timing.seed_probe_ms;
		return DSB_OK;
	}
	if (dbg) { HIPCHK(hipStreamSynchronize(c->stream)); fprintf(stderr, "[dsb] seed probe done\n"); }
	unsigned slots = (unsigned)c->n_slots; if (slots > n - n_heavy) slots = (unsigned)(n - n_heavy);
	{
		uint32_t *dbgp = dbg ? c->dbg_dev : nullptr;
		if (dbg) memset(c->dbg_host, 0, 32 * 65536 * sizeof(uint32_t));
		const bool grp = s.max_len <= DSB_GROUP_MAX_LEN && !c->knobs.no_group;
		const bool anc_k = use_scan && !dbg && !grp && c->knobs.anchor_kernel && c->arena_anc.base && c->n_slots_anc > 0 && c->arena_anc.anc_cap == c->arena.anc_cap
		                   && c->d_arec && c->cap_arec >= n && c->d_apool && n > n_heavy;
		if (anc_k) {
			unsigned ga = (unsigned)c->n_slots_anc; if (ga > n - n_heavy) ga = (unsigned)(n - n_heavy);
			hipLaunchKernelGGL(k_anchor, dim3(ga), dim3(64), 0, c->stream, dx1, (const DsbReadDesc *)s.d_rd, (uint32_t)n, (uint32_t)n_heavy, (const uint32_t *)c->d_order, c->d_bin, c->arena_anc,
			                   c->d_counters + 14, c->d_seeds, (const DsbSeedInfo *)c->d_sinfo, c->d_arec, c->d_apool, c->d_counters + 15, (uint32_t)c->cap_apool, (unsigned long long *)(c->d_counters + 16));
		}
		launch_classify(k_classify, c, c->stream, slots, dx1, s, (uint32_t)n, nullptr, (const uint32_t *)c->d_order, c->arena, c->d_counters, dbgp, (uint32_t)n_heavy, 0u, 0, use_scan,
		                anc_k ? c->d_arec : nullptr, anc_k ? c->d_apool : nullptr);
		HIPCHK(hipEventRecord(c->ev_cls, c->stream));
		HIPCHK(hipEventRecord(c->ev_cls_wait, c->stream));
		if (n_heavy) { HIPCHK(hipStreamWaitEvent(c->stream, c->ev_heavy, 0)); if (c->timing.n_heavy_mw) HIPCHK(hipStreamWaitEvent(c->stream, c->ev_heavy3, 0)); }
		if (dbg) {
			for (int sec = 0; sec < 60; sec++) {
				if (hipStreamQuery(c->stream) == hipSuccess) break;
				usleep(1000000);
				if (sec % 5 == 4) {
					fprintf(stderr, "[dsb] classify still running after %d s; slot: code steps read\n", sec + 1);
					for (unsigned sI = 0; sI < slots && sI < 24; sI++) fprintf(stderr, "   slot %u: %u %u %u\n", sI, c->dbg_host[4 * sI], c->dbg_host[4 * sI + 1], c->dbg_host[4 * sI + 2]);
				}
			}
		}
	}
	if (dx1.heavy_limit) {
		DsbDevIndex dxh = dx1; dxh.heavy_limit = 0;
		unsigned gh = (unsigned)(c->n_slots + c->n_extra); if (gh > 256u) gh = 256u;
		hipLaunchKernelGGL(k_collect_retry, dim3((unsigned)((n + 255) / 256)), dim3(256), 0, c->stream, (const DsbReadOut *)c->d_rout, (uint32_t)n, c->d_heavy, c->d_counters + 12, DSB_ST_HEAVY, 0);
		hipLaunchKernelGGL(k_classify_heavy<8>, dim3(gh), dim3(64 * 8), 0, c->stream, dxh, (const DsbReadDesc *)s.d_rd, 0u, (const unsigned int *)(c->d_counters + 12), (const uint32_t *)c->d_heavy, c->d_bin,
		                   (const uint64_t *)c->d_bits, c->arena, c->d_counters + 13, c->d_rout, c->d_hout, c->d_counters + 1, (uint32_t)c->cap_hout, 0u,
		                   (unsigned long long *)(c->d_counters + 16 + 8), (const uint64_t *)c->d_pk, use_scan ? c->d_seeds : (DsbSeed *)nullptr, (const DsbSeedInfo *)c->d_sinfo);
	}
	DsbDevIndex dx2 = c->dx; dx2.sms_cap = c->arena_big.sms_cap; dx2.heavy_limit = 0; dx2.step_limit = step_limit > 0xffffffffu / 16 ? 0xffffffffu : step_limit * 16u;
	const int retry_mask = DSB_ST_SMS_OVF | DSB_ST_ANC_OVF | DSB_ST_HIT_OVF | DSB_ST_TIMEOUT;
	hipLaunchKernelGGL(k_collect_retry, dim3((unsigned)((n + 255) / 256)), dim3(256), 0, c->stream, (const DsbReadOut *)c->d_rout, (uint32_t)n, c->d_score, c->d_counters + 6, retry_mask, 0);
	launch_classify(k_classify_second, c, c->stream, (unsigned)c->n_slots_big, dx2, s, 0u, (const unsigned int *)(c->d_counters + 6), (const uint32_t *)c->d_score, c->arena_big, c->d_counters + 7, nullptr, 0u, 0u, 2, use_scan);
	HIPCHK(hipEventRecord(c->ev[3], c->stream));
	if (turn && !c->knobs.turn_whole_run) { HIPCHK(hipEventSynchronize(c->ev_cls_wait)); turn->unlock(); }
	HIPCHK(hipEventSynchronize(c->ev[3]));
	{
		unsigned int cnt[2] = {0, 0};
		HIPCHK(hipMemcpy(cnt, c->d_counters, 8, hipMemcpyDeviceToHost));
		if (cnt[1] > c->cap_hout) {
			const size_t new_cap = 2 * (size_t)cnt[1] + 4096;
			DsbHitOut *nh = nullptr;
			if (hipMalloc((void **)&nh, new_cap * sizeof(DsbHitOut)) != hipSuccess) return DSB_ENOMEM;
			HIPCHK(hipMemcpy(nh, c->d_hout, c->cap_hout * sizeof(DsbHitOut), hipMemcpyDeviceToDevice));
			hipFree(c->d_hout); c->d_hout = nh; c->cap_hout = new_cap;
			hipLaunchKernelGGL(k_collect_retry, dim3((unsigned)((n + 255) / 256)), dim3(256), 0, c->stream, (const DsbReadOut *)c->d_rout, (uint32_t)n, c->d_score, c->d_counters + 8, DSB_ST_OUT_OVF, 0);
			launch_classify(k_classify_second, c, c->stream, (unsigned)c->n_slots_big, dx2, s, 0u, (const unsigned int *)(c->d_counters + 8), (const uint32_t *)c->d_score, c->arena_big, c->d_counters + 9, nullptr, 0u, 0u, 2, use_scan);
			HIPCHK(hipStreamSynchronize(c->stream));
			unsigned int n3 = 0; HIPCHK(hipMemcpy(&n3, c->d_counters + 8, 4, hipMemcpyDeviceToHost));
			c->timing.n_regrow = n3;
		}
	}
	const DsbBatchView hits = {c->stream, c->d_rout, c->d_hout, c->d_counters, c->cap_hout, s.d_rd, (uint32_t)n};
	if (int rc = reductions_run(c, hits)) return rc;
	if (dbg) {
		static const char *nm[10] = {"seed_vector", "fast_classify", "resolve_tree", "slow+resolve", "hash_build", "sdp_middle", "sdp_right", "sdp_left", "sort/filter", "primary"};
		double tot[10] = {0}, all = 0; unsigned sl = (unsigned)c->n_slots; if (sl > n) sl = (unsigned)n;
		double sub[4] = {0};
		for (unsigned sI = 0; sI < sl; sI++) { for (int i = 0; i < 10; i++) { tot[i] += c->dbg_host[4 * 65536 + 14 * sI + i]; all += c->dbg_host[4 * 65536 + 14 * sI + i]; } for (int i = 0; i < 4; i++) sub[i] += c->dbg_host[4 * 65536 + 14 * sI + 10 + i]; }
		fprintf(stderr, "[dsb] inside sdp_right (ms, -DDSB_TIMERS builds): sdp_match %.1f  dp %.1f  combine %.1f | fast_classify commit phase %.1f\n", sub[0] / 1e3, sub[1] / 1e3, sub[2] / 1e3, sub[3] / 1e3);
		{ double tx[10] = {0}; for (unsigned sI = 0; sI < sl; sI++) for (int i = 0; i < 10; i++) tx[i] += c->dbg_host[8 * 65536 + 10 * sI + i];
		  fprintf(stderr, "[dsb] fine (ms, -DDSB_TIMERS builds): table build %.1f  probe %.1f  block DP: old predecessors %.1f, inside the block %.1f  sdp_match in sdp_left %.1f  dp in sdp_left %.1f  gap-per-lane phase of sdp_middle %.1f | of the old predecessors: beyond the first 64 (sdp_batch_old) %.1f in %.0f blocks; rounds over the first 64: %.0f\n",
		          tx[0] / 1e3, tx[1] / 1e3, tx[2] / 1e3, tx[6] / 100.0 / 1e3, tx[3] / 1e3, tx[4] / 1e3, tx[5] / 1e3, tx[9] / 100.0 / 1e3, tx[7], tx[8]); }
		{
			size_t worst = 0; uint64_t wsum = 0;
			for (size_t r = 0; r < n && r < 65536; r++) { uint64_t sm = 0; for (int i = 0; i < 10; i++) sm += c->dbg_host[16 * 65536 + 14 * r + i]; if (sm > wsum) { wsum = sm; worst = r; } }
			fprintf(stderr, "[dsb] slowest read %zu: %.1f ms:", worst, wsum / 1e3);
			for (int i = 0; i < 10; i++) fprintf(stderr, " %s %.1f", nm[i], c->dbg_host[16 * 65536 + 14 * worst + i] / 1e3);
			fprintf(stderr, " | in right/left: sdp_match %.1f dp %.1f combine %.1f\n", c->dbg_host[16 * 65536 + 14 * worst + 10] / 1e3, c->dbg_host[16 * 65536 + 14 * worst + 11] / 1e3, c->dbg_host[16 * 65536 + 14 * worst + 12] / 1e3);
		}
		fprintf(stderr, "[dsb] classify stage time (wave-seconds, %% of total %.2f s):", all / 1e6);
		for (int i = 0; i < 10; i++) fprintf(stderr, " %s %.1f%%", nm[i], 100.0 * tot[i] / (all > 0 ? all : 1));
		fprintf(stderr, "\n");
	}
	HIPCHK(hipGetLastError());
	hipEventElapsedTime(&c->timing.encode_ms, c->ev[0], c->ev[1]);
	hipEventElapsedTime(&c->timing.order_ms, c->ev[1], c->ev_order);
	hipEventElapsedTime(&c->timing.seed_probe_ms, c->ev_order, c->ev[2]);
	hipEventElapsedTime(&c->timing.classify_ms, c->ev[2], c->ev_cls);
	hipEventElapsedTime(&c->timing.tail_ms, c->ev_cls, c->ev[3]);
	c->timing.n_early = c->n_early;
	hipEventElapsedTime(&c->timing.total_ms, c->ev[0], c->ev[3]);
	unsigned long long wk[12] = {0};
	HIPCHK(hipMemcpy(&c->p1, c->d_counters + 2, 8, hipMemcpyDeviceToHost));
	HIPCHK(hipMemcpy(&c->timing.n_retry, c->d_counters + 6, 4, hipMemcpyDeviceToHost));
	{
		unsigned int h[4] = {0, 0, 0, 0};
		HIPCHK(hipMemcpy(h, c->d_counters + 12, sizeof h, hipMemcpyDeviceToHost));
		c->timing.n_requeue = h[0]; c->timing.anc_pool_asked = h[3]; c->timing.anc_pool_cap = c->cap_apool;
	}
	if (c->timing.tail_ms > 3.0f && c->timing.n_requeue == 0 && c->timing.n_retry == 0 && c->timing.n_early) {
		if (c->mw_reads < 64) c->mw_reads = c->mw_reads ? c->mw_reads * 2 : 16;
		c->mw_grown = true; c->mw_calm = 0;
	} else if (c->timing.tail_ms < 0.5f && !c->mw_grown && c->mw_reads && c->timing.n_early && ++c->mw_calm >= 4) c->mw_reads = 0;
	HIPCHK(hipMemcpy(wk, c->d_counters + 16, 96, hipMemcpyDeviceToHost));
	c->timing.windows = s.total_windows; c->timing.probes_t1 = c->p1; c->timing.bases = s.total_bases;
	c->timing.seed_scan = use_scan ? 1 : 0;
	if (use_scan) {
		unsigned long long pc[2] = {0, 0};
		HIPCHK(hipMemcpy(pc, c->d_counters + 40, 16, hipMemcpyDeviceToHost));
		c->timing.windows = pc[0]; c->timing.probes_t1 = pc[1];
	}
	c->timing.n_occ = wk[0] + wk[4] + wk[8]; c->timing.n_mem = wk[1] + wk[5] + wk[9]; c->timing.n_sa = wk[2] + wk[6] + wk[10]; c->timing.ref_bases = wk[3] + wk[7] + wk[11];
	c->timing.main_occ = wk[0]; c->timing.main_mem = wk[1]; c->timing.main_sa = wk[2]; c->timing.main_ref_bases = wk[3];
	return DSB_OK;
}

extern "C" int dsb_batch_fetch(dsb_ctx *c, dsb_result *out)
{
	if (!c || !out) return DSB_EINVAL;
	HIPCHK(hipSetDevice(c->device));
	const size_t n = c->in[c->cur].n_reads;
	c->h_rout.resize(n); c->res_reads.resize(n);
	unsigned int cnt[2] = {0, 0};
	if (n) {
		HIPCHK(hipMemcpyAsync(cnt, c->d_counters, 8, hipMemcpyDeviceToHost, c->stream));
		HIPCHK(hipMemcpyAsync(c->h_rout.data(), c->d_rout, n * sizeof(DsbReadOut), hipMemcpyDeviceToHost, c->stream));
		HIPCHK(hipStreamSynchronize(c->stream));
	}
	const size_t nh = dsb_hits_out(cnt[1], c->cap_hout);
	c->h_hout.resize(nh);
	if (nh) HIPCHK(hipMemcpyAsync(c->h_hout.data(), c->d_hout, nh * sizeof(DsbHitOut), hipMemcpyDeviceToHost, c->stream));
	static_assert(sizeof(DsbHitOut) == sizeof(dsb_hit), "dsb_hit mirrors DsbHitOut");
	int worst = DSB_OK;
	for (size_t i = 0; i < n; i++) {
		const DsbReadOut &r = c->h_rout[i];
		dsb_read_result &o = c->res_reads[i];
		o.first = r.first; o.n = r.n; o.fast = r.fast & 1u; o.device_us = r.fast >> 1; o.n_anc = r.n_anc;
		o.status = r.status ? (DSB_ECAP * 256 - r.status) : 0;
		if (r.status) worst = DSB_ECAP;
		if (dsb_hits_cut(r.first, r.n, nh)) { o.n = 0; o.first = 0; }
	}
	if (int rc = reductions_fetch(c, n, nh != 0)) return rc;
	out->reads = c->res_reads.data(); out->hits = reinterpret_cast<const dsb_hit *>(c->h_hout.data()); out->n_hits = nh;
	return worst;
}

extern "C" int dsb_classify_batch(dsb_ctx *c, const dsb_read *reads, size_t n, dsb_result *out)
{
	int rc;
	if ((rc = dsb_batch_upload(c, reads, n))) return rc;
	if ((rc = dsb_batch_run(c))) return rc;
	return dsb_batch_fetch(c, out);
}

extern "C" int dsb_batch_timing(const dsb_ctx *c, dsb_timing *t) { if (!c || !t) return DSB_EINVAL; *t = c->timing; return DSB_OK; }

extern "C" int dsb_batch_exist_bits(dsb_ctx *c, size_t read, int strand, uint8_t *out, size_t cap, uint32_t *n_out)
{
	if (!c || read >= c->in[c->cur].n_reads) return DSB_EINVAL;
	HIPCHK(hipSetDevice(c->device));
	const InSlot &sl = c->in[c->cur];
	const DsbReadDesc &d = sl.h_rd[read];
	if (n_out) *n_out = d.n_win;
	if (cap < d.n_win) return DSB_EINVAL;
	if (!c->bits_valid && sl.n_words_total) {
		uint64_t waves = (sl.n_words_total + DSB_PROBE_UN - 1) / DSB_PROBE_UN; unsigned blocks = (unsigned)((waves + 3) / 4);
		if (blocks > 256u * 32u) blocks = 256u * 32u;
		hipLaunchKernelGGL(k_build_wd, dim3((unsigned)sl.n_reads), dim3(256), 0, c->stream, sl.d_rd, c->d_wd);
		hipLaunchKernelGGL(k_seed_probe, dim3(blocks), dim3(256), 0, c->stream, c->dx, (const DsbReadDesc *)sl.d_rd, (const DsbWordDesc *)c->d_wd, sl.n_words_total, c->d_pk, c->d_bits,
		                   (unsigned long long *)nullptr, c->d_summ, c->summ_shift);
		HIPCHK(hipStreamSynchronize(c->stream));
		c->bits_valid = true;
	}
	std::vector<uint64_t> wv(d.n_words);
	if (d.n_words) HIPCHK(hipMemcpy(wv.data(), c->d_bits + d.bit_off + (strand ? 0 : d.n_words), d.n_words * 8, hipMemcpyDeviceToHost));
	for (uint32_t i = 0; i < d.n_win; i++) out[i] = (uint8_t)((wv[i >> 6] >> (i & 63)) & 1);
	return DSB_OK;
}

__global__ void __launch_bounds__(64) k_seed_dump(DsbDevIndex x, DsbReadDesc d, uint8_t *bin, const uint64_t *bits, int strand, DsbSeed *out, uint32_t *n_out)
{
	__shared__ DsbDevIndex sx;
	__shared__ uint32_t lds_cnt[4];
	if (threadIdx.x == 0) sx = x;
	__syncthreads();
	__shared__ dsb_g64::WCtx s_w;
	dsb_g64::WCtxL &w = *(dsb_g64::WCtxL *)&s_w;
	w.x = (dsb_g64::DsbXP)&sx; w.L = d.len; w.status = 0; w.dbg = nullptr; w.anc_cap = 0; w.wtab = nullptr;
// ... 158 lines not shown
```

include/desamba_amd.h:

```cpp
#ifndef DESAMBA_AMD_H
#define DESAMBA_AMD_H
#include <stddef.h>
#include <stdint.h>

#ifdef __cplusplus
extern "C" {
#endif

#define DSB_OK        0
#define DSB_EIO      -1
#define DSB_ENODEV   -2
#define DSB_ENOMEM   -3
#define DSB_EINVAL   -4
#define DSB_ECAP     -5

typedef struct dsb_index dsb_index;
typedef struct dsb_ctx dsb_ctx;
typedef struct dsb_multi dsb_multi;

typedef struct {
	int L_min_matching;
	int min_score;
	int max_sec_N;
	int n_slots;
// ... 3 lines not shown
	int reserved;
	uint64_t max_batch_bases;
} dsb_opts;

typedef struct {
	const char *name;
	const char *seq;
	const char *qual;
	uint32_t len;
} dsb_read;

typedef struct {
	uint32_t ref_ID, t_st, t_ed, q_st, q_ed, sum_score, indel;
	uint8_t direction, primary, pri_index, pad;
} dsb_hit;

typedef struct {
	uint32_t first, n;
	int32_t status;
	uint32_t fast;
	uint32_t device_us;
	uint32_t n_anc;
} dsb_read_result;

typedef struct {
	const dsb_read_result *reads;
	const dsb_hit *hits;
	size_t n_hits;
} dsb_result;

typedef struct { uint32_t offset, len; uint8_t top; uint8_t pad[3]; } dsb_seed;

typedef struct {
	float encode_ms, seed_probe_ms, classify_ms, total_ms;
	uint64_t windows;
	uint64_t probes_t1;
	uint64_t bases;
	float order_ms;
	float tail_ms;
	uint32_t n_early;
	uint32_t n_retry;
	uint32_t n_regrow;
	uint32_t seed_scan;
	uint64_t n_occ;
	uint64_t n_mem;
	uint64_t n_sa;
	uint64_t ref_bases;
	uint64_t main_occ, main_mem, main_sa, main_ref_bases;
	uint32_t n_heavy_mw;
	uint32_t n_requeue;
	uint64_t upload_bytes;
	uint64_t anc_pool_asked;
	uint64_t anc_pool_cap;
} dsb_timing;

typedef struct {
	uint64_t n_bases, n_refs, n_kmer, n_unitig, n_rows;
	double parse_s, sort_s, graph_s, walk_s, rows_s, tables_s, write_s, total_s;
	uint64_t budget_bytes;
	uint64_t peak_device_bytes;
	uint32_t ranges_kmers, ranges_unitig_numbers, ranges_rows, ranges_exist;
	uint64_t spilled_bytes;
} dsb_build_stats;
int  dsb_index_build(const char *kmer_srt, const char *fasta, const char *out_dir, int device, dsb_build_stats *stats);

int  dsb_index_open(const char *dir, dsb_index **idx);
void dsb_index_close(dsb_index *idx);
uint64_t    dsb_index_n_ref(const dsb_index *idx);
const char *dsb_index_ref_name(const dsb_index *idx, uint32_t ref_ID);
uint64_t    dsb_index_ref_len(const dsb_index *idx, uint32_t ref_ID);
int         dsb_index_ek_len(const dsb_index *idx);
int dsb_index_prefix_interval(const dsb_index *idx, uint32_t prefix, int form, uint64_t *sp, uint64_t *ep);
uint64_t dsb_index_occ_host(const dsb_index *idx, uint64_t r, uint8_t *c);

int  dsb_device_count(void);
int  dsb_ctx_create(dsb_index *idx, int device_id, const dsb_opts *opts, dsb_ctx **ctx);
void dsb_ctx_destroy(dsb_ctx *ctx);
void dsb_ctx_reset_history(dsb_ctx *ctx);
void dsb_ctx_reload_env(dsb_ctx *ctx);
void dsb_ctx_set_history(dsb_ctx *ctx, uint32_t max_len_before);
int  dsb_ctx_use_synthetic_filter(dsb_ctx *ctx, uint64_t table_bytes, double fill);
int  dsb_synthetic_filter_bit(int which, uint64_t bit, double fill);
int  dsb_ctx_select_slot(dsb_ctx *ctx, int slot);

int  dsb_ctx_create_multi(dsb_index *idx, const int *device_ids, int n_dev, const dsb_opts *opts, dsb_multi **m);
void dsb_multi_destroy(dsb_multi *m);
int  dsb_multi_n(const dsb_multi *m);
dsb_ctx *dsb_multi_ctx(dsb_multi *m, int i);
void dsb_multi_reset_history(dsb_multi *m);
uint32_t dsb_multi_last_calls(const dsb_multi *m, int i);
int  dsb_multi_classify_batch(dsb_multi *m, const dsb_read *reads, size_t n, dsb_result *out);
typedef struct { uint64_t start, end; uint32_t hist_max_before; int32_t rank; } dsb_chunk;
int  dsb_shard_plan(const uint32_t *lengths, size_t n, int world, uint64_t chunk_bases, uint32_t chunk_reads, dsb_chunk *out, size_t cap, size_t *n_out);

int  dsb_classify_batch(dsb_ctx *ctx, const dsb_read *reads, size_t n, dsb_result *out);

int  dsb_batch_upload(dsb_ctx *ctx, const dsb_read *reads, size_t n);
int  dsb_batch_upload_text(dsb_ctx *ctx, const char *text, size_t text_len, const uint64_t *seq_off, const uint32_t *seq_len, size_t n);
void *dsb_host_alloc(size_t bytes);
void  dsb_host_free(void *p);
int   dsb_host_cpus(void);
long dsb_batch_upload_fastq(dsb_ctx *ctx, const char *path, size_t skip, size_t max_reads);
int  dsb_batch_run(dsb_ctx *ctx);
int  dsb_batch_fetch(dsb_ctx *ctx, dsb_result *out);
int  dsb_batch_timing(const dsb_ctx *ctx, dsb_timing *t);
int  dsb_batch_seeds(dsb_ctx *ctx, size_t read, int strand, dsb_seed *out, size_t cap, uint32_t *n, uint32_t *total_score);
// ... 110 lines not shown
```

Measured before the change: 173,800.

## Add prefix-max score bound to prune predecessor scans in sparse DP

Keeps a per-node running prefix maximum of DP scores (pmax) in a new per-slot arena buffer and fills it in the serial, batched and multi-wave extension paths. During backward predecessor scans, a node stops early once its current best (or seed score) reaches the bound pmax[hi]+len, because no earlier predecessor can do better. This cuts the number of predecessors visited per node. The cost is extra global writes and reads of pmax, a wave prefix-max scan, extra ballots, and more arena memory. It is on by default and can be disabled with DSB_DP_BOUND.

```diff
diff --git a/__graft_entry__.py b/__graft_entry__.py
--- a/__graft_entry__.py
+++ b/__graft_entry__.py
@@ -88,6 +88,21 @@
     emu64 = os.path.join(emu_dir, "libdsbemu64.so")
     if not _newer(emu64, [emu_src, os.path.join(emu_dir, "dsb_emu_shim.h"), os.path.join(emu_dir, "emu_simt.cpp")] + deps):
         _run([os.path.join(emu_dir, "build_emu64.sh")])
+    dp_src = os.path.join(emu_dir, "emu_dp_bound.cpp")
+    if os.path.exists(dp_src):
+        inc_flags = ["-DDSB_HOST_EMU", "-I" + CSRC, "-I" + os.path.join(ROOT, "include"), "-I" + emu_dir]
+        dp_deps = [dp_src, os.path.join(emu_dir, "dsb_emu_shim.h")] + deps
+        dp1 = os.path.join(emu_dir, "libdsbemu_dp.so")
+        if not _newer(dp1, dp_deps):
+            _run(["g++", "-std=c++17", "-O2", "-fno-strict-aliasing", "-fPIC", "-shared"] + inc_flags + ["-o", dp1, dp_src])
+        dp64 = os.path.join(emu_dir, "libdsbemu_dp64.so")
+        simt = os.path.join(emu_dir, "emu_simt.cpp")
+        if not _newer(dp64, dp_deps + [simt]):
+            import tempfile
+            with tempfile.TemporaryDirectory() as tmp:
+                _run(["g++", "-std=c++17", "-O1", "-g", "-fsanitize=thread", "-fno-strict-aliasing", "-fPIC", "-DDSB_EMU_LANES=64"] + inc_flags + ["-c", dp_src, "-o", os.path.join(tmp, "dp.o")])
+                _run(["g++", "-std=c++17", "-O2", "-g", "-fPIC", "-c", simt, "-o", os.path.join(tmp, "simt.o")])
+                _run(["g++", "-shared", "-o", dp64, os.path.join(tmp, "dp.o"), os.path.join(tmp, "simt.o"), "-ldl"])
     sys.path.insert(0, ROOT)
     import desamba_amd
     L = desamba_amd.lib()
diff --git a/desamba_amd/__init__.py b/desamba_amd/__init__.py
--- a/desamba_amd/__init__.py
+++ b/desamba_amd/__init__.py
@@ -45,7 +45,7 @@
                 ("n_occ", C.c_uint64), ("n_mem", C.c_uint64), ("n_sa", C.c_uint64), ("ref_bases", C.c_uint64),
                 ("main_occ", C.c_uint64), ("main_mem", C.c_uint64), ("main_sa", C.c_uint64), ("main_ref_bases", C.c_uint64),
                 ("n_heavy_mw", C.c_uint32), ("n_requeue", C.c_uint32), ("upload_bytes", C.c_uint64),
-                ("anc_pool_asked", C.c_uint64), ("anc_pool_cap", C.c_uint64)]
+                ("anc_pool_asked", C.c_uint64), ("anc_pool_cap", C.c_uint64), ("dp_preds", C.c_uint64)]
 
 
 class DsbBuildStats(C.Structure):
diff --git a/desamba_amd/csrc/dsb_classify_dev.h b/desamba_amd/csrc/dsb_classify_dev.h
--- a/desamba_amd/csrc/dsb_classify_dev.h
+++ b/desamba_amd/csrc/dsb_classify_dev.h
@@ -75,13 +75,14 @@
 	uint32_t cmd;
 	uint32_t n0, K;
 	const DsbSms *sms;
+	const int *pmax;
 	uint32_t nd_t[8], nd_q[8], nd_l[8];
 	uint32_t cut[2][DSB_MW_MAXW];
 	int32_t best[DSB_MW_MAXW][8];
 };
 
 #define DSB_DPB 8
-struct DpBatch { uint32_t n0, K; int old_best[DSB_DPB]; uint32_t nd_t[DSB_DPB], nd_q[DSB_DPB], nd_l[DSB_DPB]; };
+struct DpBatch { uint32_t n0, K; int old_best[DSB_DPB]; uint32_t nd_t[DSB_DPB], nd_q[DSB_DPB], nd_l[DSB_DPB]; int seed[DSB_DPB]; };
 typedef DSB_LDS_AS DpBatch DpBatchL;
 
 struct SDir { DsbSeed *seed_v; uint32_t l_seed_v; uint8_t *bin_read; const uint64_t *bits; uint32_t direction, total_score; };
@@ -99,6 +100,8 @@
 	DsbAnchor *lane_anc; uint64_t *lane_spset; uint32_t *top_idx;
 	DsbChain *hit, *hit_tmp; uint32_t n_hit;
 	DsbSms *sms; uint32_t n_sms;
+	int *pmax;
+	uint32_t dp_bound;
 	uint32_t *wtab;
 	DsbScHash *sc;
 	DsbMem *mem_slow;
@@ -1933,6 +1936,10 @@
 	}
 	stopm = DSB_RFL(stopm); wnm = DSB_RFL(wnm);
 	const int32_t n0 = (int32_t)b.n0;
+	const int *const pmax = w.dp_bound ? w.pmax : nullptr;
+	int seed[DSB_DPB];
+#pragma unroll
+	for (int j = 0; j < DSB_DPB; j++) seed[j] = (int)DSB_RFL(b.seed[j]);
 	DsbSms nx[DSB_DP_UNROLL];
 #define DSB_FETCH_PREDS(dst, hi_, ng_)                                                                          \
 	_Pragma("unroll") for (int u = 0; u < DSB_DP_UNROLL; u++) {                                                 \
@@ -1960,6 +1967,8 @@
 		}
 		const int32_t hi_next = hi - ng * DSB_WAVE;
 		if (ng == DSB_DP_UNROLL && hi_next >= 0) { DSB_FETCH_PREDS(nx, hi_next, DSB_DP_UNROLL) }
+		int pm_next = 0;
+		if (pmax && hi_next >= 0) pm_next = pmax[hi_next];
 		const bool plain = wnm == 0 && !(wrapped[0] | wrapped[1] | wrapped[2] | wrapped[3]) && ng == DSB_DP_UNROLL;
 		uint32_t redo = ~stopm & ((1u << DSB_DPB) - 1u);
 		if (plain) {
@@ -2017,6 +2026,15 @@
 				if (ok && ns > best[j]) best[j] = ns;
 			}
 		}
+		if (pmax && hi_next >= 0) {
+			const int pm = (int)DSB_RFL(pm_next);
+#pragma unroll
+			for (int j = 0; j < DSB_DPB; j++) {
+				if ((stopm >> j) & 1u) continue;
+				const int need = pm + (int)nl[j];
+				if (seed[j] >= need || dsb_ballot64(best[j] >= need) != 0) stopm |= 1u << j;
+			}
+		}
 		if (stopm == (1u << DSB_DPB) - 1u) break;
 		if (ng != DSB_DP_UNROLL && hi_next >= 0) { DSB_FETCH_PREDS(nx, hi_next, DSB_DP_UNROLL) }
 		hi = hi_next; ng = DSB_DP_UNROLL;
@@ -2032,7 +2050,7 @@
 {
 	uint32_t lq[DSB_DPB], lt[DSB_DPB], dl[DSB_DPB], nq[DSB_DPB], nt[DSB_DPB], nl[DSB_DPB]; int best[DSB_DPB];
 	uint32_t stopm = 0, wnm = 0, preds = 0;
-	const uint32_t K = mw->K; const DsbSms *const sms = mw->sms;
+	const uint32_t K = mw->K; const DsbSms *const sms = mw->sms; const int *const pmax = mw->pmax;
 #pragma unroll
 	for (int j = 0; j < DSB_DPB; j++) {
 		DsbSms nd; nd.t_pos = mw->nd_t[j]; nd.q_pos = mw->nd_q[j]; nd.len = mw->nd_l[j]; nd.score = 0;
@@ -2074,6 +2092,8 @@
 				wrapped[u] = dsb_ballot64((int)(A[u] | B[u] | C[u]) < 0) != 0;
 			}
 			if (hi - W * step >= 0) { DSB_FETCH_PREDS_MW(nx, hi - W * step) }
+			int pm_next = 0;
+			if (pmax && hi - step >= 0) pm_next = pmax[hi - step];
 			const bool plain = wnm == 0 && !(wrapped[0] | wrapped[1] | wrapped[2] | wrapped[3]);
 			uint32_t redo = ~stopm & ((1u << DSB_DPB) - 1u);
 			if (plain) {
@@ -2125,6 +2145,15 @@
 					if (ok && ns > v[j]) v[j] = ns;
 				}
 			}
+			if (pmax && hi - step >= 0) {
+				const int pm = (int)DSB_RFL(pm_next);
+#pragma unroll
+				for (int j = 0; j < DSB_DPB; j++) {
+					if (((stopm | cutm) >> j) & 1u) continue;
+					const int need = pm + (int)nl[j]; const int have = MAXV(best[j], v[j]);
+					if (dsb_ballot64(have >= need) != 0) cutm |= 1u << j;
+				}
+			}
 		}
 		const uint32_t par = round & 1u;
 		if (lane == 0) mw->cut[par][wv] = cutm;
@@ -2160,10 +2189,11 @@
 			const DsbSms g_ = w.sms[cur + j];
 			b.nd_t[j] = g_.t_pos; b.nd_q[j] = g_.q_pos; b.nd_l[j] = g_.len;
 		}
+		for (uint32_t j = 0; j < DSB_DPB; j++) b.seed[j] = j < bK ? (int)b.nd_l[j] : 0;
 		if (w.mw && bn0 >= DSB_MW_MIN_PREDS) {
 			DsbMw *mw = w.mw;
 			if (DSB_LANE < DSB_DPB) { const int sj = (uint32_t)DSB_LANE < b.K ? DSB_LANE : 0; mw->nd_t[DSB_LANE] = b.nd_t[sj]; mw->nd_q[DSB_LANE] = b.nd_q[sj]; mw->nd_l[DSB_LANE] = b.nd_l[sj]; }
-			if (DSB_LANE == 0) { mw->cmd = (uint32_t)MODE; mw->n0 = b.n0; mw->K = b.K; mw->sms = w.sms; }
+			if (DSB_LANE == 0) { mw->cmd = (uint32_t)MODE; mw->n0 = b.n0; mw->K = b.K; mw->sms = w.sms; mw->pmax = w.dp_bound ? w.pmax : nullptr; }
 			block_sync();
 			uint32_t preds = 0;
 			sdp_batch_old_mw<MODE>(mw, w.ring, w.red, DSB_LANE, 0, w.n_waves, &preds);
@@ -2251,14 +2281,15 @@
 	}
 	uint64_t left = dsb_ballot64(!done);
 	TX0(w, t_deep);
+	if (hi >= 0 && left && w.dp_bound) { const int pm = w.pmax[hi]; left = dsb_ballot64(!done && best < pm + (int)nl); }
 	if (hi >= 0 && left) {
 		TXC(w, 7);
 		DpBatchL &b = *w.dpb;
 		while (left) {
 			int id[DSB_DPB]; uint32_t K = 0;
 			for (int j = 0; j < DSB_DPB; j++) { id[j] = -1; if (left) { id[j] = (int)__builtin_ctzll(left); left &= left - 1; K++; } }
-			for (int j = 0; j < DSB_DPB; j++) if (lane == id[j]) { b.nd_t[j] = cs.t_pos; b.nd_q[j] = cs.q_pos; b.nd_l[j] = cs.len; }
-			if (lane == 0) { b.n0 = (uint32_t)hi + 1; b.K = K; for (uint32_t j = K; j < DSB_DPB; j++) { b.nd_t[j] = 0; b.nd_q[j] = 0; b.nd_l[j] = 0; } }
+			for (int j = 0; j < DSB_DPB; j++) if (lane == id[j]) { b.nd_t[j] = cs.t_pos; b.nd_q[j] = cs.q_pos; b.nd_l[j] = cs.len; b.seed[j] = best; }
+			if (lane == 0) { b.n0 = (uint32_t)hi + 1; b.K = K; for (uint32_t j = K; j < DSB_DPB; j++) { b.nd_t[j] = 0; b.nd_q[j] = 0; b.nd_l[j] = 0; b.seed[j] = 0; } }
 			wave_sync();
 			sdp_batch_old<MODE, false>(w, b);
 			wave_sync();
@@ -2598,12 +2629,14 @@
 	fill_window(w, ref, 1000 + 128);
 	wave_sync();
 	DsbSms *p = push_sms(w);
+	if (w.dp_bound) w.pmax[0] = score_ori;
 	p->score = score_ori; p->q_pos = c_h->q_ed; p->t_pos = c_h->t_ed; p->len = 1 - 9;
 	ring_put(w, 0, p->t_pos, p->q_pos, p->len, p->score);
 	uint32_t best_t = c_h->t_ed, best_q = c_h->q_ed, best_len = (uint32_t)(1 - 9);
 	NodeBlock nb; nb.base = 0; nb.valid = 0;
 	DpBatchL &db = *w.dpb; db.n0 = 0; db.K = 0;
 	uint32_t bn0 = 0, bK = 0;
+	int pm_run = score_ori;
 	uint32_t current_sms = 1;
 	uint64_t t_offset_global = x->refinfo[c_h->ref_ID].seq_offset, t_length = x->refinfo[c_h->ref_ID].seq_l;
 	uint32_t c_t_offset = c_h->t_ed - 3;
@@ -2643,6 +2676,7 @@
 		SUB1(w, 11);
 		TXC(w, 8);
 		c_sms->score = max_score;
+		pm_run = MAXV(pm_run, max_score); if (w.dp_bound) w.pmax[current_sms - 1] = pm_run;
 		{ uint4 r_; r_.x = cs.t_pos; r_.y = cs.q_pos; r_.z = cs.len; r_.w = (uint32_t)max_score; ring_st(ring, (current_sms - 1) & (DSB_RING - 1), r_); }
 		SUB0(w);
 		bool comb = (int)cs.len >= 8 && combine_chain(c_st, chain_ID, sc_hash, cs.t_pos - cs.q_pos, false, cs.q_pos, &combined) == true;
@@ -2656,9 +2690,10 @@
 			score_ori = total_max_score; max_sms_id = 0;
 			w.n_sms = 0;
 			p = push_sms(w); n_sms = 1;
-			p->score = total_max_score; p->q_pos = c_h->q_ed; p->t_pos = c_h->t_ed; p->len = -9;
+			if (w.dp_bound) w.pmax[0] = total_max_score;
+	p->score = total_max_score; p->q_pos = c_h->q_ed; p->t_pos = c_h->t_ed; p->len = -9;
 			ring_put(w, 0, p->t_pos, p->q_pos, p->len, p->score);
-			best_t = c_h->t_ed; best_q = c_h->q_ed; best_len = (uint32_t)(-9); nb.valid = 0; db.K = 0; bK = 0;
+			best_t = c_h->t_ed; best_q = c_h->q_ed; best_len = (uint32_t)(-9); nb.valid = 0; db.K = 0; bK = 0; pm_run = total_max_score;
 			current_sms = 1;
 			c_t_offset = c_h->t_ed;
 			continue;
@@ -2683,12 +2718,14 @@
 	fill_window(w, ref, 1000 + 128);
 	wave_sync();
 	DsbSms *p = push_sms(w);
+	if (w.dp_bound) w.pmax[0] = score_ori;
 	p->score = score_ori; p->q_pos = c_h->q_st; p->t_pos = c_h->t_st;
 	ring_put(w, 0, p->t_pos, p->q_pos, 0, p->score);
 	uint32_t best_t = c_h->t_st, best_q = c_h->q_st;
 	NodeBlock nb; nb.base = 0; nb.valid = 0;
 	DpBatchL &db = *w.dpb; db.n0 = 0; db.K = 0;
 	uint32_t bn0 = 0, bK = 0;
+	int pm_run = score_ori;
 	uint32_t current_sms = 1;
 	uint64_t t_offset_global = x->refinfo[c_h->ref_ID].seq_offset;
 	uint32_t c_t_offset = c_h->t_st + 3;
@@ -2730,6 +2767,7 @@
 		int max_score = sdp_best_pred_b<2>(w, db, cs, (int32_t)current_sms - 1, nb, n_sms, ring, steps, bn0, bK);
 		TX1(w, 4, t_ld);
 		c_sms->score = max_score;
+		pm_run = MAXV(pm_run, max_score); if (w.dp_bound) w.pmax[current_sms - 1] = pm_run;
 		{ uint4 r_; r_.x = cs.t_pos; r_.y = cs.q_pos; r_.z = cs.len; r_.w = (uint32_t)max_score; ring_st(ring, (current_sms - 1) & (DSB_RING - 1), r_); }
 		if ((int)cs.len >= 8 && combine_chain(c_st, chain_ID, sc_hash, cs.t_pos - cs.q_pos, true, cs.q_pos + cs.len, &combined) == true) {
 			int c_len = cs.len;
@@ -2740,9 +2778,10 @@
 			score_ori = total_max_score; max_sms_id = 0;
 			w.n_sms = 0;
 			p = push_sms(w); n_sms = 1;
-			p->score = total_max_score; p->q_pos = c_h->q_st; p->t_pos = c_h->t_st;
+			if (w.dp_bound) w.pmax[0] = total_max_score;
+	p->score = total_max_score; p->q_pos = c_h->q_st; p->t_pos = c_h->t_st;
 			ring_put(w, 0, p->t_pos, p->q_pos, 0, p->score);
-			best_t = c_h->t_st; best_q = c_h->q_st; nb.valid = 0; db.K = 0; bK = 0;
+			best_t = c_h->t_st; best_q = c_h->q_st; nb.valid = 0; db.K = 0; bK = 0; pm_run = total_max_score;
 			current_sms = 1;
 			c_t_offset = c_h->t_st;
 			continue;
@@ -2759,16 +2798,31 @@
 #define DSB_EXT_NEXT 0
 #define DSB_EXT_STOP 1
 #define DSB_EXT_MERGED 2
+DV int wave_prefix_max_i(int v)
+{
+	for (int d = 1; d < DSB_WAVE; d <<= 1) { const int t = (int)dsb_shfl_var((uint32_t)v, DSB_LANE - d); if (DSB_LANE >= d && t > v) v = t; }
+	return v;
+}
 struct ExtState { int total_max_score; uint32_t best_t, best_q, best_len; uint32_t steps; int merge_score; uint32_t merge_len; DsbChain *combined; };
 template <int MODE>
-DV int ext_block(WCtxL &w, ExtState &e, const uint32_t n0, const uint32_t m, DsbChain *c_st, int chain_ID, DsbScHash *sc_hash, const uint32_t step_limit)
+DV int ext_block_scores(WCtxL &w, const uint32_t n0, const uint32_t m, DsbSms &cs)
 {
 	const int lane = DSB_LANE; DsbSms *const sms = w.sms;
 	const bool mine = (uint32_t)lane < m;
-	DsbSms cs; cs.t_pos = cs.q_pos = cs.len = cs.score = 0;
+	cs.t_pos = cs.q_pos = cs.len = cs.score = 0;
 	if (mine) cs = sms[n0 + lane];
 	const int sc = sdp_block_scores<MODE>(w, n0, m, cs);
 	if (mine) sms[n0 + lane].score = (uint32_t)sc;
+	if (w.dp_bound) { const int pm = wave_prefix_max_i(mine ? sc : (-2147483647 - 1)), carry = w.pmax[n0 - 1]; if (mine) w.pmax[n0 + lane] = MAXV(pm, carry); }
+	return sc;
+}
+template <int MODE>
+DV int ext_block(WCtxL &w, ExtState &e, const uint32_t n0, const uint32_t m, DsbChain *c_st, int chain_ID, DsbScHash *sc_hash, const uint32_t step_limit)
+{
+	const int lane = DSB_LANE;
+	const bool mine = (uint32_t)lane < m;
+	DsbSms cs;
+	const int sc = ext_block_scores<MODE>(w, n0, m, cs);
 	const bool cand = mine && (int)cs.len >= 8 && combine_test(c_st, chain_ID, sc_hash, (int)(cs.t_pos - cs.q_pos), MODE == 2, (int)(MODE == 2 ? cs.q_pos + cs.len : cs.q_pos));
 	const uint64_t cmask = dsb_ballot64(cand);
 	wave_sync();
@@ -2797,6 +2851,7 @@
 	fill_window(w, ref, 1000 + 128);
 	wave_sync();
 	DsbSms *p = push_sms(w);
+	if (w.dp_bound) w.pmax[0] = score_ori;
 	p->score = score_ori; p->q_pos = c_h->q_ed; p->t_pos = c_h->t_ed; p->len = 1 - 9;
 	ExtState e; e.total_max_score = score_ori; e.best_t = c_h->t_ed; e.best_q = c_h->q_ed; e.best_len = (uint32_t)(1 - 9);
 	e.steps = w.steps; e.combined = nullptr; e.merge_score = 0; e.merge_len = 0;
@@ -2845,7 +2900,8 @@
 			score_ori = e.total_max_score;
 			w.n_sms = 0;
 			p = push_sms(w); n_sms = 1;
-			p->score = e.total_max_score; p->q_pos = c_h->q_ed; p->t_pos = c_h->t_ed; p->len = -9;
+			if (w.dp_bound) w.pmax[0] = e.total_max_score;
+	p->score = e.total_max_score; p->q_pos = c_h->q_ed; p->t_pos = c_h->t_ed; p->len = -9;
 			e.best_t = c_h->t_ed; e.best_q = c_h->q_ed; e.best_len = (uint32_t)(-9);
 			current_sms = 1;
 			c_t_offset = c_h->t_ed;
@@ -2870,6 +2926,7 @@
 	fill_window(w, ref, 1000 + 128);
 	wave_sync();
 	DsbSms *p = push_sms(w);
+	if (w.dp_bound) w.pmax[0] = score_ori;
 	p->score = score_ori; p->q_pos = c_h->q_st; p->t_pos = c_h->t_st; p->len = 0;
 	ExtState e; e.total_max_score = score_ori; e.best_t = c_h->t_st; e.best_q = c_h->q_st; e.best_len = 0;
 	e.steps = w.steps; e.combined = nullptr; e.merge_score = 0; e.merge_len = 0;
@@ -2921,7 +2978,8 @@
 			score_ori = e.total_max_score;
 			w.n_sms = 0;
 			p = push_sms(w); n_sms = 1;
-			p->score = e.total_max_score; p->q_pos = c_h->q_st; p->t_pos = c_h->t_st; p->len = 0;
+			if (w.dp_bound) w.pmax[0] = e.total_max_score;
+	p->score = e.total_max_score; p->q_pos = c_h->q_st; p->t_pos = c_h->t_st; p->len = 0;
 			e.best_t = c_h->t_st; e.best_q = c_h->q_st;
 			current_sms = 1;
 			c_t_offset = c_h->t_st;
diff --git a/desamba_amd/csrc/dsb_ctx.h b/desamba_amd/csrc/dsb_ctx.h
--- a/desamba_amd/csrc/dsb_ctx.h
+++ b/desamba_amd/csrc/dsb_ctx.h
@@ -29,6 +29,7 @@
 	int upload_threads = 0, seed_scan = -1, heavy_mw = -1, heavy_first = 0;
 	bool heavy_preds_set = false; uint32_t heavy_preds = 0;
 	uint64_t em_hash_mask = ~0ull;
+	bool dp_bound = true;
 	bool anchor_kernel = true; long anc_pool_rt = 0;
 	bool scan_look_set = false; DsbScanLook scan_look;
 	std::string order_file;
diff --git a/desamba_amd/csrc/dsb_device.h b/desamba_amd/csrc/dsb_device.h
--- a/desamba_amd/csrc/dsb_device.h
+++ b/desamba_amd/csrc/dsb_device.h
@@ -34,6 +34,7 @@
 	uint32_t sms_cap;
 	uint32_t step_limit;
 	uint32_t heavy_limit;
+	uint32_t dp_bound;
 };
 
 struct DsbSeed { uint32_t offset; uint16_t len, top; };
@@ -55,7 +56,7 @@
 struct DsbScHash { uint16_t next; uint16_t seed_ID; };
 
 struct DsbHitOut { uint32_t ref_ID, t_st, t_ed, q_st, q_ed, sum_score, indel; uint8_t direction, primary, pri_index, pad; };
-struct DsbReadOut { uint32_t first, n; int32_t status; uint32_t fast; uint32_t n_anc, pad; };
+struct DsbReadOut { uint32_t first, n; int32_t status; uint32_t fast; uint32_t n_anc, dp_preds; };
 struct DsbAncRec { uint32_t off, n, lsteps, use; };
 
 struct DsbReadDesc {
@@ -73,7 +74,7 @@
 
 struct DsbSlotArena {
 	uint8_t *base; size_t stride;
-	size_t off_seeds, off_anc, off_anc_tmp, off_hit, off_hit_tmp, off_sms, off_sc, off_mem, off_spset, off_scorev,
+	size_t off_seeds, off_anc, off_anc_tmp, off_hit, off_hit_tmp, off_sms, off_pmax, off_sc, off_mem, off_spset, off_scorev,
 	       off_sortkey, off_sortidx, off_win, off_lane_anc, off_lane_sp, off_top, off_round;
 	uint32_t max_len;
 	uint32_t sms_cap;
diff --git a/desamba_amd/csrc/dsb_gpu.hip b/desamba_amd/csrc/dsb_gpu.hip
--- a/desamba_amd/csrc/dsb_gpu.hip
+++ b/desamba_amd/csrc/dsb_gpu.hip
@@ -391,7 +391,7 @@
 	w.seeds = (DsbSeed *)(slot + ar.off_seeds);
 	w.anc = (DsbAnchor *)(slot + ar.off_anc); w.anc_tmp = (DsbAnchor *)(slot + ar.off_anc_tmp);
 	w.hit = (DsbChain *)(slot + ar.off_hit); w.hit_tmp = (DsbChain *)(slot + ar.off_hit_tmp);
-	w.sms = (DsbSms *)(slot + ar.off_sms);
+	w.sms = (DsbSms *)(slot + ar.off_sms); w.pmax = (int *)(slot + ar.off_pmax); w.dp_bound = x.dp_bound;
 	w.sc = (DsbScHash *)(slot + ar.off_sc); w.wtab = lds_wtab;
 	w.mem_slow = (DsbMem *)(slot + ar.off_mem);
 	w.spset = (uint64_t *)(slot + ar.off_spset);
@@ -479,7 +479,7 @@
 		}
 		if (w.dbg && lane == 0) { w.dbg[0] = 200; if (r < 65536u) for (int i = 0; i < 14; i++) dbg[16 * 65536 + 14 * r + i] = (uint32_t)((w.tacc[i] - tacc0[i]) / 100); }
 		if (lane == 0) { DsbReadOut ro; ro.first = first; ro.n = n_out; ro.status = w.status | (w.status ? (w.stage << 8) : 0);
-			ro.fast = fast | ((uint32_t)((wall_clock64() - t_start) / 100) << 1); ro.n_anc = w.n_anc; ro.pad = 0; rout[r] = ro; }
+			ro.fast = fast | ((uint32_t)((wall_clock64() - t_start) / 100) << 1); ro.n_anc = w.n_anc; ro.dp_preds = w.dp_preds; rout[r] = ro; }
 		}
 	}
 }
@@ -618,7 +618,7 @@
 		w.seeds = (DsbSeed *)(slot + ar.off_seeds);
 		w.anc = (DsbAnchor *)(slot + ar.off_anc); w.anc_tmp = (DsbAnchor *)(slot + ar.off_anc_tmp);
 		w.hit = (DsbChain *)(slot + ar.off_hit); w.hit_tmp = (DsbChain *)(slot + ar.off_hit_tmp);
-		w.sms = (DsbSms *)(slot + ar.off_sms);
+		w.sms = (DsbSms *)(slot + ar.off_sms); w.pmax = (int *)(slot + ar.off_pmax); w.dp_bound = x.dp_bound;
 		w.sc = (DsbScHash *)(slot + ar.off_sc); w.wtab = lds_wtab;
 		w.mem_slow = (DsbMem *)(slot + ar.off_mem);
 		w.spset = (uint64_t *)(slot + ar.off_spset);
@@ -664,7 +664,7 @@
 				hout[first + i] = o;
 			}
 			if (lane == 0) { DsbReadOut ro; ro.first = first; ro.n = n_out; ro.status = w.status | (w.status ? (w.stage << 8) : 0);
-				ro.fast = fast | ((uint32_t)((wall_clock64() - t_start) / 100) << 1); ro.n_anc = w.n_anc; ro.pad = 0; rout[r] = ro; }
+				ro.fast = fast | ((uint32_t)((wall_clock64() - t_start) / 100) << 1); ro.n_anc = w.n_anc; ro.dp_preds = w.dp_preds; rout[r] = ro; }
 		} else {
 			__builtin_amdgcn_s_setprio(3);
 			for (;;) {
@@ -809,6 +809,7 @@
 	k.heavy_mw = getenv("DSB_HEAVY_MW") ? (int)num("DSB_HEAVY_MW", 0) : -1;
 	k.heavy_first_set = getenv("DSB_HEAVY_FIRST") != nullptr; k.heavy_first = (int)num("DSB_HEAVY_FIRST", 0);
 	k.anchor_kernel = num("DSB_ANCHOR_KERNEL", 1) != 0;
+	k.dp_bound = num("DSB_DP_BOUND", 1) != 0;
 	if (getenv("DSB_EM_HASH_BITS")) { const long b = num("DSB_EM_HASH_BITS", 64); k.em_hash_mask = b >= 64 ? ~0ull : b < 1 ? 1ull : (1ull << b) - 1; }
 	k.anc_pool_rt = num("DSB_ANC_POOL_RT", 0); if (getenv("DSB_ANC_POOL_RT") && k.anc_pool_rt < 1) k.anc_pool_rt = 1;
 	if (const char *e = getenv("DSB_HEAVY_PREDS")) { k.heavy_preds_set = true; k.heavy_preds = (uint32_t)strtoul(e, nullptr, 10); }
@@ -1023,6 +1024,7 @@
 	a.off_hit = o;     o += al256((size_t)hit_cap * sizeof(DsbChain));
 	a.off_hit_tmp = o; o += al256((size_t)hit_cap * sizeof(DsbChain));
 	a.off_sms = o;     o += f * al256((size_t)sms_cap * sizeof(DsbSms));
+	a.off_pmax = o;    o += f * al256((size_t)sms_cap * sizeof(int));
 	a.off_sc = o;      o += f * al256((size_t)(256 + 2 * 400 + 64) * sizeof(DsbScHash));
 	a.off_mem = o;     o += f * al256((size_t)DSB_MEMSLOW_CAP * sizeof(DsbMem));
 	a.off_spset = o;   o += al256((size_t)DSB_SPHASH * 8);
@@ -1388,7 +1390,7 @@
 	c->bits_valid = !use_scan; c->seeds_valid = use_scan;
 	uint32_t step_limit = DSB_STEP_LIMIT;
 	if (c->knobs.step_limit_rt > 0) step_limit = (uint32_t)c->knobs.step_limit_rt;
-	DsbDevIndex dx1 = c->dx; dx1.sms_cap = c->arena.sms_cap; dx1.step_limit = step_limit;
+	DsbDevIndex dx1 = c->dx; dx1.sms_cap = c->arena.sms_cap; dx1.step_limit = step_limit; dx1.dp_bound = c->knobs.dp_bound ? 1u : 0u;
 	dx1.heavy_limit = DSB_HEAVY_PREDS;
 	if (dbg) dx1.heavy_limit = 0;
 	if (c->knobs.heavy_preds_set) dx1.heavy_limit = c->knobs.heavy_preds;
@@ -1472,7 +1474,7 @@
 		                   (const uint64_t *)c->d_bits, c->arena, c->d_counters + 13, c->d_rout, c->d_hout, c->d_counters + 1, (uint32_t)c->cap_hout, 0u,
 		                   (unsigned long long *)(c->d_counters + 16 + 8), (const uint64_t *)c->d_pk, use_scan ? c->d_seeds : (DsbSeed *)nullptr, (const DsbSeedInfo *)c->d_sinfo);
 	}
-	DsbDevIndex dx2 = c->dx; dx2.sms_cap = c->arena_big.sms_cap; dx2.heavy_limit = 0; dx2.step_limit = step_limit > 0xffffffffu / 16 ? 0xffffffffu : step_limit * 16u;
+	DsbDevIndex dx2 = c->dx; dx2.sms_cap = c->arena_big.sms_cap; dx2.dp_bound = dx1.dp_bound; dx2.heavy_limit = 0; dx2.step_limit = step_limit > 0xffffffffu / 16 ? 0xffffffffu : step_limit * 16u;
 	const int retry_mask = DSB_ST_SMS_OVF | DSB_ST_ANC_OVF | DSB_ST_HIT_OVF | DSB_ST_TIMEOUT;
 	hipLaunchKernelGGL(k_collect_retry, dim3((unsigned)((n + 255) / 256)), dim3(256), 0, c->stream, (const DsbReadOut *)c->d_rout, (uint32_t)n, c->d_score, c->d_counters + 6, retry_mask, 0);
 	launch_classify(k_classify_second, c, c->stream, (unsigned)c->n_slots_big, dx2, s, 0u, (const unsigned int *)(c->d_counters + 6), (const uint32_t *)c->d_score, c->arena_big, c->d_counters + 7, nullptr, 0u, 0u, 2, use_scan);
@@ -1567,8 +1569,10 @@
 	if (nh) HIPCHK(hipMemcpyAsync(c->h_hout.data(), c->d_hout, nh * sizeof(DsbHitOut), hipMemcpyDeviceToHost, c->stream));
 	static_assert(sizeof(DsbHitOut) == sizeof(dsb_hit), "dsb_hit mirrors DsbHitOut");
 	int worst = DSB_OK;
+	c->timing.dp_preds = 0;
 	for (size_t i = 0; i < n; i++) {
 		const DsbReadOut &r = c->h_rout[i];
+		c->timing.dp_preds += r.dp_preds;
 		dsb_read_result &o = c->res_reads[i];
 		o.first = r.first; o.n = r.n; o.fast = r.fast & 1u; o.device_us = r.fast >> 1; o.n_anc = r.n_anc;
 		o.status = r.status ? (DSB_ECAP * 256 - r.status) : 0;
diff --git a/include/desamba_amd.h b/include/desamba_amd.h
--- a/include/desamba_amd.h
+++ b/include/desamba_amd.h
@@ -79,6 +79,7 @@
 	uint64_t upload_bytes;
 	uint64_t anc_pool_asked;
 	uint64_t anc_pool_cap;
+	uint64_t dp_preds;
 } dsb_timing;
 
 typedef struct {
```

Measured after the change: 174,500, median of 6. About the same (+0.4%).
